# jneem/nnnoiseless

Hardware: NVIDIA H100
Metric: 48kHz mono frames/sec (480-sample) (higher is better)
Workload: dtype f32

## Files before the change

### nnnoiseless_b200/build.py

```python
import os
import subprocess
import sys

HERE = os.path.dirname(os.path.abspath(__file__))
CSRC = os.path.join(HERE, "csrc")
VARIANT = os.environ.get("NNB_VARIANT", "")
OBJ = os.path.join(HERE, "_obj" + ("_" + VARIANT if VARIANT else ""))
LIBDIR = os.path.join(HERE, "lib")
LIB = os.path.join(LIBDIR, "libnnnoiseless_b200%s.so" % ("_" + VARIANT if VARIANT else ""))
VARIANT_FLAGS = {"": [], "prof": ["-DPITCH_PROFILE", "-DRNN_TC_PROFILE"]}[VARIANT]
WEIGHTS = os.path.join(HERE, "data", "weights.rnn")
BINDIR = os.path.join(HERE, "bin")
CLI = os.path.join(BINDIR, "nnnoiseless-b200")
CLI_SRC = os.path.join(HERE, "..", "cli", "nnnoiseless_cli.cpp")
NVCC = os.environ.get("NVCC", "/usr/local/cuda/bin/nvcc")

ARCH = ["-gencode", "arch=compute_90a,code=sm_90a"]
COMMON = ["-O3", "-std=c++17", "-lineinfo", "-Xcompiler", "-fPIC", "-Xptxas", "-v"]

UNITS = [
    ("exact.cu", ["-fmad=false"]),
    ("pitch.cu", ["-fmad=false"]),
    ("train.cu", ["-fmad=false"]),
    ("spectral.cu", []),
    ("spectral_warp.cu", []),
    ("rnn.cu", ["-DRNN_RT=256", "-DRNN_UNROLL=8"]),
    ("rnn_mma.cu", []),
    ("rnn_tc.cu", []),
    ("frontend.cu", []),
    ("host.cu", []),
]
HEADERS = ["common.cuh", "fft480.cuh", "model.hpp", "audio_io.hpp", os.path.join("..", "..", "include", "rnnoise.h")]


def _newer(target, deps):
    if not os.path.exists(target):
        return True
    t = os.path.getmtime(target)
    return any(os.path.getmtime(d) > t for d in deps)


def build(force=False, verbose=False):
    os.makedirs(OBJ, exist_ok=True)
    os.makedirs(LIBDIR, exist_ok=True)
    hdrs = [os.path.join(CSRC, h) for h in HEADERS] + [os.path.abspath(__file__)]
    objs = []
    logs = []
    for src, extra in UNITS:
        s = os.path.join(CSRC, src)
        o = os.path.join(OBJ, src + ".o")
        objs.append(o)
        if force or _newer(o, [s] + hdrs):
            cmd = [NVCC] + ARCH + COMMON + extra + VARIANT_FLAGS + os.environ.get("NNB_EXTRA_NVCC", "").split() + ["-c", s, "-o", o]
            r = subprocess.run(cmd, capture_output=True, text=True)
            logs.append(r.stderr)
            if r.returncode != 0:
                sys.stderr.write(r.stdout + r.stderr)
                raise RuntimeError("nvcc failed on " + src)
            if verbose:
                sys.stderr.write(r.stderr)
    s = os.path.join(CSRC, "model.cpp")
    o = os.path.join(OBJ, "model.cpp.o")
    objs.append(o)
    if force or _newer(o, [s, WEIGHTS] + hdrs):
        cmd = ["g++", "-O2", "-std=c++17", "-fPIC", '-DNNB_WEIGHTS_PATH="%s"' % WEIGHTS, "-c", s, "-o", o]
        subprocess.run(cmd, check=True)
    s = os.path.join(CSRC, "audio_io.cpp")
    o = os.path.join(OBJ, "audio_io.cpp.o")
    objs.append(o)
    if force or _newer(o, [s] + hdrs):
        subprocess.run(["g++", "-O2", "-std=c++17", "-fPIC", "-Wall", "-c", s, "-o", o], check=True)
    if force or _newer(LIB, objs):
        cmd = [NVCC] + ARCH + ["-shared", "-o", LIB] + objs
        subprocess.run(cmd, check=True)
    os.makedirs(BINDIR, exist_ok=True)
    if not VARIANT and (force or _newer(CLI, [CLI_SRC, LIB] + hdrs)):
        cmd = ["g++", "-O2", "-std=c++17", "-Wall", CLI_SRC, "-o", CLI, "-L" + LIBDIR, "-lnnnoiseless_b200",
               "-Wl,-rpath,$ORIGIN/../lib"]
        subprocess.run(cmd, check=True)
    with open(os.path.join(OBJ, "ptxas.log"), "a") as f:
        f.write("".join(logs))
    return LIB


if __name__ == "__main__":
    print(build(force="--force" in sys.argv, verbose=True))
```

### nnnoiseless_b200/csrc/common.cuh

```cuda
#pragma once
#include <cuda_runtime.h>
#include <stdint.h>

namespace nnb {

constexpr int FRAME_SIZE = 480;
constexpr int WINDOW_SIZE = 960;
constexpr int FREQ_SIZE = 481;
constexpr int PITCH_MIN_PERIOD = 60;
constexpr int PITCH_MAX_PERIOD = 768;
constexpr int PITCH_FRAME_SIZE = 960;
constexpr int PITCH_BUF_SIZE = PITCH_MAX_PERIOD + PITCH_FRAME_SIZE;
constexpr int NB_BANDS = 22;
constexpr int CEPS_MEM = 8;
constexpr int NB_DELTA_CEPS = 6;
constexpr int NB_FEATURES = 42;
constexpr int MAX_NEURONS = 128;
constexpr int NB_BINS_BANDED = 400;
constexpr int BT_LANES = 96;

constexpr int HIST_SLOTS = 8;
constexpr int HIST_CAP = HIST_SLOTS * FRAME_SIZE;
constexpr int PIPE_DEPTH = 4;

__host__ __device__ inline int hist_base(int slot) { return (slot * FRAME_SIZE + (HIST_CAP - (PITCH_BUF_SIZE - FRAME_SIZE))) % HIST_CAP; }

struct DeviceTables {
    float window[WINDOW_SIZE];
    float dct[NB_BANDS * NB_BANDS];
    float wnorm;
    float tansig[201 + 3];
    float2 tw480[480];
    float2 tw960[FREQ_SIZE + 3];
    float band_frac[NB_BINS_BANDED];
    int32_t band_of[NB_BINS_BANDED];
    int32_t band_start[NB_BANDS];
    int16_t bt_bin[800];
    float bt_w[800];
    int16_t bt_lane_start[BT_LANES + 1];
    int16_t bt_band_lane[NB_BANDS + 1];
    int16_t bt_lane_band[BT_LANES];
    float2 twl[15][32];
    int16_t bp_seg[32];
    int16_t bp_b0[32];
    int16_t bp_n[32];
    int16_t bp_rot[32];
    int16_t bp_off[32];
    float bp_inv[32];
};
constexpr int BP_MAXBINS = 22;

struct DeviceLayer {
    int ni, nn, np, act;
    const float* w;
    const float* wh;
    const float* bias;
};

struct DeviceModel {
    DeviceLayer input_dense, vad_gru, noise_gru, denoise_gru, denoise_output, vad_output;
    int state_size;
};

constexpr int MMA_MAX_CHUNKS = 28;
struct MmaPhase {
    int nchunks;
    int ntiles;
    const uint2* wfrag;
    const float* bias;
    short col[MMA_MAX_CHUNKS];
};
struct DeviceModelMma {
    MmaPhase dense, vad_zr, vad_h, vad_out, noise_zr, noise_h, den_zr, den_h, out;
    int nd, nv, nn, ndn;
    int act_dense, act_vad, act_noise, act_den, act_out, act_vadout;
    int c_feat, c_dense, c_vad, c_noise, c_den, c_rh;
    int kp;
    int hs;
    int state_size;
};

struct BatchBuffers {
    int n_streams;
    float* hist;
    float* hp_mem;
    float* synth_mem;
    float* ceps_mem;
    int32_t* ceps_id;
    int32_t* last_period;
    float* last_gain;
    float* gru_state;
    float* lastg;
    float2* X;
    float2* P;
    float* ex;
    float* ep;
    float* exp;
    float* features;
    int32_t* silence;
    int32_t* pitch;
    float* gains;
    float* vad;
    unsigned long long* pitch_stats;
};

constexpr int TRAIN_ROW = NB_FEATURES + 2 * NB_BANDS + 1;
struct TrainLaneParams {
    float signal_gain, noise_gain;
    float sig_a[2], sig_b[2], noise_a[2], noise_b[2];
    int32_t band_lp;
};
struct TrainBuffers {
    int n_lanes;
    TrainLaneParams* params;
    float* resp_mem;
    int32_t* vad_count;
    float* vad;
    int32_t* cutoff;
};

struct DeviceGuard {
    int prev = -1, want = -1;
    cudaError_t err = cudaSuccess;
    explicit DeviceGuard(int dev) : want(dev) {
        err = cudaGetDevice(&prev);
        if (err == cudaSuccess && prev != dev) err = cudaSetDevice(dev);
    }
    ~DeviceGuard() {
        if (prev >= 0 && prev != want) cudaSetDevice(prev);
    }
    DeviceGuard(const DeviceGuard&) = delete;
    DeviceGuard& operator=(const DeviceGuard&) = delete;
};

cudaError_t launch_hp_filter(const BatchBuffers& b, const void* in, bool pcm16, long stream_stride, long sample_stride, int slot,
                             cudaStream_t st);
cudaError_t launch_pitch(const BatchBuffers& b, int slot, int force_exact, cudaStream_t st);
cudaError_t launch_analysis(const BatchBuffers& b, const DeviceTables* tab, int slot, cudaStream_t st);
cudaError_t launch_synthesis(const BatchBuffers& b, const DeviceTables* tab, void* out, bool pcm16, long stream_stride, long sample_stride,
                             float* vad_out, cudaStream_t st);
cudaError_t launch_analysis_warp(const BatchBuffers& b, const DeviceTables* tab, int slot, cudaStream_t st);
cudaError_t launch_synthesis_warp(const BatchBuffers& b, const DeviceTables* tab, void* out, bool pcm16, long stream_stride,
                                  long sample_stride, float* vad_out, cudaStream_t st);
cudaError_t launch_rnn(const BatchBuffers& b, const DeviceModel& m, const DeviceTables* tab, cudaStream_t st);
cudaError_t launch_rnn_mma(const BatchBuffers& b, const DeviceModelMma& m, const DeviceTables* tab, cudaStream_t st);

constexpr int TC_PHASES = 9;
enum { PH_DENSE = 0, PH_VAD_ZR, PH_VAD_H, PH_VAD_OUT, PH_NOISE_ZR, PH_NOISE_H, PH_DEN_ZR, PH_DEN_H, PH_OUT };
struct TcPhase {
    int n;
    int nk;
    uint32_t w_off;
    uint32_t b_off;
    short chunk[16];
};
constexpr int TC_MAX_SLABS = 64;
struct TcSlab {
    uint32_t off, bytes;
    short phase, kc0, kc1;
};
struct DeviceModelTc {
    TcPhase ph[TC_PHASES];
    int nd, nv, nn, ndn;
    int p_d, p_v, p_n, p_dn;
    int o_dense, o_vad, o_noise, o_den, o_rh;
    int act_dense, act_vad, act_noise, act_den, act_out, act_vadout;
    int state_size;
    const unsigned char* blob;
    uint32_t blob_bytes, table_off;
    int n_slabs;
    short slab0[TC_PHASES + 1];
    TcSlab slab[TC_MAX_SLABS];
};

struct UploadedTc {
    DeviceModelTc dm{};
    unsigned char* d_blob = nullptr;
    size_t smem_bytes = 0;
    bool ok = false;
};

struct HostModel;
int upload_model_tc(const HostModel& hm, UploadedTc* u, cudaStream_t st);
cudaError_t launch_rnn_tc(const BatchBuffers& b, const UploadedTc& u, cudaStream_t st);

cudaError_t launch_train_front(const BatchBuffers& b, const TrainBuffers& tb, int set, const float* signal, const float* noise,
                               long stream_stride, int slot, cudaStream_t st);
cudaError_t launch_train_rows(const BatchBuffers& b, const TrainBuffers& tb, int set, float* rows, long lane_stride, cudaStream_t st);

}
```

### nnnoiseless_b200/csrc/host.cu

```cuda
#include <atomic>
#include <cmath>
#include <cstdio>
#include <cstdlib>
#include <cstring>
#include <mutex>
#include <new>
#include <string>
#include <algorithm>
#include <utility>
#include <vector>

#include <cuda_fp16.h>

#include "../../include/rnnoise.h"
#include "common.cuh"
#include "model.hpp"

using namespace nnb;

struct RNNModel {
    HostModel m;
};

namespace {

thread_local std::string g_err;
std::atomic<unsigned long long> g_launches{0};

int fail(const std::string& what, cudaError_t e = cudaSuccess) {
    g_err = what;
    if (e != cudaSuccess) {
        g_err += ": ";
        g_err += cudaGetErrorString(e);
    }
    return -1;
}

}

namespace nnb {
int set_error(const std::string& what) { return fail(what); }
void count_launches(int n) { g_launches.fetch_add((unsigned long long)n, std::memory_order_relaxed); }
}

namespace {

#define ON_DEVICE(dev)                                                   \
    DeviceGuard guard__(dev);                                            \
    if (guard__.err != cudaSuccess) return fail("cudaSetDevice", guard__.err)

#define CK(call)                                         \
    do {                                                 \
        cudaError_t e__ = (call);                        \
        if (e__ != cudaSuccess) return fail(#call, e__); \
    } while (0)

}
namespace nnb {
extern const float kTansigTable[201] = {
    0.000000f, 0.039979f, 0.079830f, 0.119427f, 0.158649f, 0.197375f, 0.235496f, 0.272905f, 0.309507f, 0.345214f, 0.379949f,
    0.413644f, 0.446244f, 0.477700f, 0.507977f, 0.537050f, 0.564900f, 0.591519f, 0.616909f, 0.641077f, 0.664037f, 0.685809f,
    0.706419f, 0.725897f, 0.744277f, 0.761594f, 0.777888f, 0.793199f, 0.807569f, 0.821040f, 0.833655f, 0.845456f, 0.856485f,
    0.866784f, 0.876393f, 0.885352f, 0.893698f, 0.901468f, 0.908698f, 0.915420f, 0.921669f, 0.927473f, 0.932862f, 0.937863f,
    0.942503f, 0.946806f, 0.950795f, 0.954492f, 0.957917f, 0.961090f, 0.964028f, 0.966747f, 0.969265f, 0.971594f, 0.973749f,
    0.975743f, 0.977587f, 0.979293f, 0.980869f, 0.982327f, 0.983675f, 0.984921f, 0.986072f, 0.987136f, 0.988119f, 0.989027f,
    0.989867f, 0.990642f, 0.991359f, 0.992020f, 0.992631f, 0.993196f, 0.993718f, 0.994199f, 0.994644f, 0.995055f, 0.995434f,
    0.995784f, 0.996108f, 0.996407f, 0.996682f, 0.996937f, 0.997172f, 0.997389f, 0.997590f, 0.997775f, 0.997946f, 0.998104f,
    0.998249f, 0.998384f, 0.998508f, 0.998623f, 0.998728f, 0.998826f, 0.998916f, 0.999000f, 0.999076f, 0.999147f, 0.999213f,
    0.999273f, 0.999329f, 0.999381f, 0.999428f, 0.999472f, 0.999513f, 0.999550f, 0.999585f, 0.999617f, 0.999646f, 0.999673f,
    0.999699f, 0.999722f, 0.999743f, 0.999763f, 0.999781f, 0.999798f, 0.999813f, 0.999828f, 0.999841f, 0.999853f, 0.999865f,
    0.999875f, 0.999885f, 0.999893f, 0.999902f, 0.999909f, 0.999916f, 0.999923f, 0.999929f, 0.999934f, 0.999939f, 0.999944f,
    0.999948f, 0.999952f, 0.999956f, 0.999959f, 0.999962f, 0.999965f, 0.999968f, 0.999970f, 0.999973f, 0.999975f, 0.999977f,
    0.999978f, 0.999980f, 0.999982f, 0.999983f, 0.999984f, 0.999986f, 0.999987f, 0.999988f, 0.999989f, 0.999990f, 0.999990f,
    0.999991f, 0.999992f, 0.999992f, 0.999993f, 0.999994f, 0.999994f, 0.999994f, 0.999995f, 0.999995f, 0.999996f, 0.999996f,
    0.999996f, 0.999997f, 0.999997f, 0.999997f, 0.999997f, 0.999997f, 0.999998f, 0.999998f, 0.999998f, 0.999998f, 0.999998f,
    0.999998f, 0.999999f, 0.999999f, 0.999999f, 0.999999f, 0.999999f, 0.999999f, 0.999999f, 0.999999f, 0.999999f, 0.999999f,
    0.999999f, 0.999999f, 0.999999f, 1.000000f, 1.000000f, 1.000000f, 1.000000f, 1.000000f, 1.000000f, 1.000000f, 1.000000f,
    1.000000f, 1.000000f, 1.000000f,
};
}
namespace {
const int kEband5ms[NB_BANDS] = {0, 1, 2, 3, 4, 5, 6, 7, 8, 10, 12, 14, 16, 20, 24, 28, 34, 40, 48, 60, 78, 100};

void build_tables(DeviceTables* t) {
    std::memset(t, 0, sizeof(*t));
    const double pi = 3.14159265358979323846264338327950288;
    for (int i = 0; i < FRAME_SIZE; i++) {
        double s = std::sin(0.5 * pi * ((double)i + 0.5) / (double)FRAME_SIZE);
        float w = (float)std::sin(0.5 * pi * s * s);
        t->window[i] = w;
        t->window[WINDOW_SIZE - i - 1] = w;
    }
    volatile float acc = 0.0f;
    for (int i = 0; i < WINDOW_SIZE; i++) acc = acc + t->window[i] * t->window[i];
    t->wnorm = 1.0f / acc;
    for (int i = 0; i < NB_BANDS; i++)
        for (int j = 0; j < NB_BANDS; j++) {
            float v = (float)std::cos(((double)i + 0.5) * (double)j * pi / (double)NB_BANDS);
            if (j == 0) v *= std::sqrt(0.5f);
            t->dct[i * NB_BANDS + j] = v;
        }
    for (int i = 0; i < 201; i++) t->tansig[i] = kTansigTable[i];
    for (int k = 0; k < 480; k++)
        t->tw480[k] = make_float2((float)std::cos(-2.0 * pi * (double)k / 480.0), (float)std::sin(-2.0 * pi * (double)k / 480.0));
    for (int k = 0; k <= 480; k++)
        t->tw960[k] = make_float2((float)std::cos(-2.0 * pi * (double)k / 960.0), (float)std::sin(-2.0 * pi * (double)k / 960.0));
    for (int i = 0; i < NB_BANDS; i++) t->band_start[i] = kEband5ms[i] << 2;
    for (int i = 0; i < NB_BANDS - 1; i++) {
        int band_size = (kEband5ms[i + 1] - kEband5ms[i]) << 2;
        for (int j = 0; j < band_size; j++) {
            int idx = (kEband5ms[i] << 2) + j;
            t->band_frac[idx] = (float)j / (float)band_size;
            t->band_of[idx] = i;
        }
    }
    int nterm = 0, lane = 0;
    for (int b = 0; b < NB_BANDS; b++) {
        const int first = nterm;
        if (b > 0)
            for (int i = t->band_start[b - 1]; i < t->band_start[b]; i++) {
                t->bt_bin[nterm] = (int16_t)i;
                t->bt_w[nterm++] = t->band_frac[i];
            }
        if (b < NB_BANDS - 1)
            for (int i = t->band_start[b]; i < t->band_start[b + 1]; i++) {
                t->bt_bin[nterm] = (int16_t)i;
                t->bt_w[nterm++] = 1.0f - t->band_frac[i];
            }
        const int n = nterm - first, lanes = (n + 8) / 9;
        t->bt_band_lane[b] = (int16_t)lane;
        for (int l = 0; l < lanes; l++) {
            t->bt_lane_band[lane] = (int16_t)b;
            t->bt_lane_start[lane++] = (int16_t)(first + (int)((long)n * l / lanes));
        }
    }
    for (int k1 = 0; k1 < 15; k1++)
        for (int b = 0; b < 32; b++) {
            const double ang = -2.0 * pi * (double)(b * k1) / 480.0;
            t->twl[k1][b] = make_float2((float)std::cos(ang), (float)std::sin(ang));
        }
    {
        int l = 0;
        for (int sgi = 0; sgi < NB_BANDS - 1; sgi++) {
            const int first = t->band_start[sgi], size = t->band_start[sgi + 1] - first;
            const int nl = size <= 16 ? 1 : (size <= 32 ? 2 : (size <= 48 ? 3 : 4));
            for (int q = 0; q < nl; q++) {
                const int lo = first + (int)((long)size * q / nl), hi = first + (int)((long)size * (q + 1) / nl);
                if (l >= 32 || hi - lo > BP_MAXBINS) {
                    fprintf(stderr, "nnnoiseless_b200: band partition broken\n");
                    abort();
                }
                static const int kRot[32] = {2, 1, 0, 0, 3, 0, 1, 0, 6, 5, 4, 0, 1, 6, 3, 0, 9, 2, 0, 12, 2, 1, 15, 3, 15, 3, 2, 2, 21, 19, 12, 4};
                t->bp_seg[l] = (int16_t)sgi;
                t->bp_b0[l] = (int16_t)lo;
                t->bp_n[l] = (int16_t)(hi - lo);
                t->bp_rot[l] = (int16_t)(kRot[l] % (hi - lo));
                t->bp_off[l] = (int16_t)(lo - first);
                t->bp_inv[l] = 1.0f / (float)size;
                l++;
            }
        }
        if (l != 32) {
            fprintf(stderr, "nnnoiseless_b200: band partition uses %d lanes\n", l);
            abort();
        }
    }
    t->bt_band_lane[NB_BANDS] = (int16_t)lane;
    t->bt_lane_start[lane] = (int16_t)nterm;
    if (lane != BT_LANES || nterm != 800) {
        fprintf(stderr, "nnnoiseless_b200: band table construction broken (%d lanes, %d terms)\n", lane, nterm);
        abort();
    }
}

struct UploadedModel {
    DeviceModel dm{};
    float* d_blob = nullptr;
};

inline int pad4(int n) { return (n + 3) & ~3; }
size_t dense_floats(const HostDense& l) { return (size_t)l.ni * pad4(l.nn) + pad4(l.nn); }
size_t gru_floats(const HostGru& l) { return (size_t)(l.ni + l.nn) * 3 * pad4(l.nn) + 3 * pad4(l.nn); }

void fill_dense(const HostModel& m, const HostDense& l, std::vector<float>& blob, size_t* off, DeviceLayer* out, float* dbase) {
    const int8_t* w = m.bytes.data() + l.w_off;
    const int8_t* b = m.bytes.data() + l.b_off;
    const int np = pad4(l.nn);
    out->ni = l.ni;
    out->nn = l.nn;
    out->np = np;
    out->act = l.act;
    out->w = dbase + *off;
    for (int j = 0; j < l.ni; j++)
        for (int o = 0; o < np; o++) blob[(*off)++] = o < l.nn ? (float)w[(size_t)j * l.nn + o] : 0.0f;
    out->wh = nullptr;
    out->bias = dbase + *off;
    for (int o = 0; o < np; o++) blob[(*off)++] = o < l.nn ? (float)b[o] : 0.0f;
}

void fill_gru(const HostModel& m, const HostGru& l, std::vector<float>& blob, size_t* off, DeviceLayer* out, float* dbase) {
    const int8_t* w = m.bytes.data() + l.w_off;
    const int8_t* r = m.bytes.data() + l.r_off;
    const int8_t* b = m.bytes.data() + l.b_off;
    const int ni = l.ni, nn = l.nn, st = 3 * nn, np = pad4(nn);
    out->ni = ni;
    out->nn = nn;
    out->np = np;
    out->act = l.act;
    auto put_rows = [&](const int8_t* src, int rows, int gate0, int ngates) {
        for (int j = 0; j < rows; j++)
            for (int g = 0; g < ngates; g++)
                for (int o = 0; o < np; o++) blob[(*off)++] = o < nn ? (float)src[(size_t)j * st + (gate0 + g) * nn + o] : 0.0f;
    };
    out->w = dbase + *off;
    put_rows(w, ni, 0, 2);
    put_rows(r, nn, 0, 2);
    out->wh = dbase + *off;
    put_rows(w, ni, 2, 1);
    put_rows(r, nn, 2, 1);
    out->bias = dbase + *off;
    for (int g = 0; g < 3; g++)
        for (int o = 0; o < np; o++) blob[(*off)++] = o < nn ? (float)b[g * nn + o] : 0.0f;
}

int upload_model(const HostModel& m, UploadedModel* um, cudaStream_t st) {
    size_t total = dense_floats(m.input_dense) + gru_floats(m.vad_gru) + gru_floats(m.noise_gru) + gru_floats(m.denoise_gru) +
                   dense_floats(m.denoise_output) + dense_floats(m.vad_output);
    std::vector<float> blob(total);
    CK(cudaMalloc(&um->d_blob, total * sizeof(float)));
    size_t off = 0;
    fill_dense(m, m.input_dense, blob, &off, &um->dm.input_dense, um->d_blob);
    fill_gru(m, m.vad_gru, blob, &off, &um->dm.vad_gru, um->d_blob);
    fill_gru(m, m.noise_gru, blob, &off, &um->dm.noise_gru, um->d_blob);
    fill_gru(m, m.denoise_gru, blob, &off, &um->dm.denoise_gru, um->d_blob);
    fill_dense(m, m.denoise_output, blob, &off, &um->dm.denoise_output, um->d_blob);
    fill_dense(m, m.vad_output, blob, &off, &um->dm.vad_output, um->d_blob);
    um->dm.state_size = m.vad_gru.nn + m.noise_gru.nn + m.denoise_gru.nn;
    CK(cudaMemcpyAsync(um->d_blob, blob.data(), total * sizeof(float), cudaMemcpyHostToDevice, st));
    CK(cudaStreamSynchronize(st));
    return 0;
}

struct UploadedMma {
    DeviceModelMma dm{};
    unsigned char* d_blob = nullptr;
};

struct Seg {
    int acol, len, recurrent, src_off;
};

inline int pad16(int n) { return (n + 15) & ~15; }
inline uint32_t pack_h2(int a, int b) {
    return (uint32_t)__half_as_ushort(__float2half((float)a)) | ((uint32_t)__half_as_ushort(__float2half((float)b)) << 16);
}

struct PhaseBuilder {
    std::vector<unsigned char> blob;
    std::vector<std::pair<MmaPhase*, std::pair<size_t, size_t>>> fixups;

    template <typename WF, typename BF>
    void add(MmaPhase* ph, const std::vector<Seg>& segs, int nout, int ngates, WF weight, BF bias) {
        const int ot = (nout + 7) / 8;
        ph->ntiles = ngates * ot;
        ph->nchunks = 0;
        std::vector<std::pair<int, int>> chunks;
        for (size_t si = 0; si < segs.size(); si++)
            for (int c = 0; c < pad16(segs[si].len); c += 16) {
                if (ph->nchunks >= MMA_MAX_CHUNKS) abort();
                ph->col[ph->nchunks++] = (short)(segs[si].acol + c);
                chunks.push_back({(int)si, c});
            }
        while (blob.size() % 16) blob.push_back(0);
        const size_t woff = blob.size();
        blob.resize(woff + (size_t)ph->nchunks * ph->ntiles * 32 * sizeof(uint2));
        uint2* wf = reinterpret_cast<uint2*>(blob.data() + woff);
        for (int kc = 0; kc < ph->nchunks; kc++) {
            const Seg& sg = segs[chunks[kc].first];
            const int r0 = chunks[kc].second;
            for (int nt = 0; nt < ph->ntiles; nt++) {
                const int gate = nt / ot, o0 = (nt % ot) * 8;
                for (int lane = 0; lane < 32; lane++) {
                    const int g = lane >> 2, t = lane & 3, n = o0 + g;
                    auto w = [&](int kr) -> int {
                        const int i = r0 + kr;
                        if (i >= sg.len || n >= nout) return 0;
                        return weight(sg, i, gate, n);
                    };
                    wf[((size_t)kc * ph->ntiles + nt) * 32 + lane] =
                        make_uint2(pack_h2(w(2 * t), w(2 * t + 1)), pack_h2(w(2 * t + 8), w(2 * t + 9)));
                }
            }
        }
        const size_t boff = blob.size();
        blob.resize(boff + (size_t)ph->ntiles * 8 * sizeof(float));
        float* bf = reinterpret_cast<float*>(blob.data() + boff);
        for (int nt = 0; nt < ph->ntiles; nt++)
            for (int j = 0; j < 8; j++) {
                const int gate = nt / ot, o = (nt % ot) * 8 + j;
                bf[nt * 8 + j] = o < nout ? (float)bias(gate, o) : 0.0f;
            }
        fixups.push_back({ph, {woff, boff}});
    }
};

int upload_model_mma(const HostModel& m, UploadedMma* um, cudaStream_t st) {
    DeviceModelMma& d = um->dm;
    const int nd = m.input_dense.nn, nv = m.vad_gru.nn, nn = m.noise_gru.nn, ndn = m.denoise_gru.nn;
    d.nd = nd; d.nv = nv; d.nn = nn; d.ndn = ndn;
    d.act_dense = m.input_dense.act; d.act_vad = m.vad_gru.act; d.act_noise = m.noise_gru.act; d.act_den = m.denoise_gru.act;
    d.act_out = m.denoise_output.act; d.act_vadout = m.vad_output.act;
    d.c_feat = 0;
    d.c_dense = pad16(NB_FEATURES);
    d.c_vad = d.c_dense + pad16(nd);
    d.c_noise = d.c_vad + pad16(nv);
    d.c_den = d.c_noise + pad16(nn);
    d.c_rh = d.c_den + pad16(ndn);
    int cols = d.c_rh + pad16(std::max(nv, std::max(nn, ndn)));
    int kp = cols;
    while ((kp / 2) % 8 != 4) kp += 2;
    d.kp = kp;
    int hs = ((nv + 7) & ~7) + ((nn + 7) & ~7) + ((ndn + 7) & ~7);
    while (hs % 32 != 8) hs++;
    d.hs = hs;
    d.state_size = nv + nn + ndn;

    const int8_t* B = m.bytes.data();
    PhaseBuilder pb;
    auto dense_w = [&](const HostDense& L) {
        return [&, B](const Seg& sg, int i, int, int n) -> int { return B[L.w_off + (size_t)(sg.src_off + i) * L.nn + n]; };
    };
    auto dense_b = [&](const HostDense& L) { return [&, B](int, int o) -> int { return B[L.b_off + o]; }; };
    auto gru_w = [&](const HostGru& L, int gate0) {
        return [&, B, gate0](const Seg& sg, int i, int gate, int n) -> int {
            const size_t st3 = (size_t)3 * L.nn;
            const size_t base = sg.recurrent ? L.r_off : L.w_off;
            return B[base + (size_t)(sg.src_off + i) * st3 + (size_t)(gate0 + gate) * L.nn + n];
        };
    };
    auto gru_b = [&](const HostGru& L, int gate0) { return [&, B, gate0](int gate, int o) -> int { return B[L.b_off + (size_t)(gate0 + gate) * L.nn + o]; }; };

    pb.add(&d.dense, {{d.c_feat, NB_FEATURES, 0, 0}}, nd, 1, dense_w(m.input_dense), dense_b(m.input_dense));
    pb.add(&d.vad_zr, {{d.c_dense, nd, 0, 0}, {d.c_vad, nv, 1, 0}}, nv, 2, gru_w(m.vad_gru, 0), gru_b(m.vad_gru, 0));
    pb.add(&d.vad_h, {{d.c_dense, nd, 0, 0}, {d.c_rh, nv, 1, 0}}, nv, 1, gru_w(m.vad_gru, 2), gru_b(m.vad_gru, 2));
    pb.add(&d.vad_out, {{d.c_vad, nv, 0, 0}}, 1, 1, dense_w(m.vad_output), dense_b(m.vad_output));
    pb.add(&d.noise_zr, {{d.c_dense, nd, 0, 0}, {d.c_vad, nv, 0, nd}, {d.c_feat, NB_FEATURES, 0, nd + nv}, {d.c_noise, nn, 1, 0}}, nn, 2,
           gru_w(m.noise_gru, 0), gru_b(m.noise_gru, 0));
    pb.add(&d.noise_h, {{d.c_dense, nd, 0, 0}, {d.c_vad, nv, 0, nd}, {d.c_feat, NB_FEATURES, 0, nd + nv}, {d.c_rh, nn, 1, 0}}, nn, 1,
           gru_w(m.noise_gru, 2), gru_b(m.noise_gru, 2));
    pb.add(&d.den_zr, {{d.c_vad, nv, 0, 0}, {d.c_noise, nn, 0, nv}, {d.c_feat, NB_FEATURES, 0, nv + nn}, {d.c_den, ndn, 1, 0}}, ndn, 2,
           gru_w(m.denoise_gru, 0), gru_b(m.denoise_gru, 0));
    pb.add(&d.den_h, {{d.c_vad, nv, 0, 0}, {d.c_noise, nn, 0, nv}, {d.c_feat, NB_FEATURES, 0, nv + nn}, {d.c_rh, ndn, 1, 0}}, ndn, 1,
           gru_w(m.denoise_gru, 2), gru_b(m.denoise_gru, 2));
    pb.add(&d.out, {{d.c_den, ndn, 0, 0}}, NB_BANDS, 1, dense_w(m.denoise_output), dense_b(m.denoise_output));

    CK(cudaMalloc(&um->d_blob, pb.blob.size()));
    for (auto& f : pb.fixups) {
        f.first->wfrag = reinterpret_cast<const uint2*>(um->d_blob + f.second.first);
        f.first->bias = reinterpret_cast<const float*>(um->d_blob + f.second.second);
    }
    CK(cudaMemcpyAsync(um->d_blob, pb.blob.data(), pb.blob.size(), cudaMemcpyHostToDevice, st));
    CK(cudaStreamSynchronize(st));
    return 0;
}

}

constexpr int kNumKernels = 5;
const char* const kKernelNames[kNumKernels] = {"hp_filter", "pitch", "analysis", "rnn", "synthesis"};
constexpr int kEvRing = 16;

struct RNNoiseBatch {
    int device = 0;
    int n_streams = 0;
    cudaStream_t st[kNumKernels] = {nullptr, nullptr, nullptr, nullptr, nullptr};
    cudaStream_t c_in = nullptr, c_out = nullptr;
    cudaEvent_t ev[kNumKernels][kEvRing];
    cudaEvent_t ev_in[kEvRing], ev_call = nullptr;
    bool events_ok = false;
    BatchBuffers buf{};
    std::vector<void*> allocs;
    DeviceTables* d_tab = nullptr;
    UploadedModel um;
    UploadedMma umm;
    UploadedTc utc;
    bool rnn_mma = false;
    bool rnn_fp32 = false;
    bool spectral_v1 = false;
    bool serial = false;
    int pitch_exact = 0;
    unsigned long long frame = 0;
    char* stage_in = nullptr;
    char* stage_out = nullptr;
    float* stage_vad = nullptr;
    size_t stage_bytes = 0;
    cudaEvent_t ev_out[8];
    int slot_ev[8];
};
constexpr int kStageSlots = 8;

namespace {

template <typename T>
int dalloc(RNNoiseBatch* b, T** p, size_t count) {
    void* q = nullptr;
    CK(cudaMalloc(&q, count * sizeof(T)));
    b->allocs.push_back(q);
    *p = reinterpret_cast<T*>(q);
    return 0;
}

BatchBuffers view(const RNNoiseBatch* b, unsigned long long f) {
    BatchBuffers v = b->buf;
    const size_t k = (size_t)(f % PIPE_DEPTH), B = (size_t)b->n_streams;
    v.X += k * B * FREQ_SIZE;
    v.P += k * B * NB_BINS_BANDED;
    v.ex += k * B * NB_BANDS;
    v.ep += k * B * NB_BANDS;
    v.exp += k * B * NB_BANDS;
    v.features += k * B * NB_FEATURES;
    v.silence += k * B;
    v.pitch += k * B;
    v.gains += k * B * NB_BANDS;
    v.vad += k * B;
    return v;
}

int sync_all(RNNoiseBatch* b) {
    for (int i = 0; i < kNumKernels; i++) CK(cudaStreamSynchronize(b->st[i]));
    CK(cudaStreamSynchronize(b->c_in));
    CK(cudaStreamSynchronize(b->c_out));
    return 0;
}

int zero_state(RNNoiseBatch* b) {
    const size_t B = (size_t)b->n_streams, D = PIPE_DEPTH;
    BatchBuffers& u = b->buf;
    const int SS = b->um.dm.state_size;
    if (sync_all(b)) return -1;
    cudaStream_t s = b->st[0];
    CK(cudaMemsetAsync(u.hist, 0, B * HIST_CAP * sizeof(float), s));
    CK(cudaMemsetAsync(u.hp_mem, 0, B * 2 * sizeof(float), s));
    CK(cudaMemsetAsync(u.synth_mem, 0, B * FRAME_SIZE * sizeof(float), s));
    CK(cudaMemsetAsync(u.ceps_mem, 0, B * CEPS_MEM * NB_BANDS * sizeof(float), s));
    CK(cudaMemsetAsync(u.ceps_id, 0, B * sizeof(int32_t), s));
    CK(cudaMemsetAsync(u.last_period, 0, B * sizeof(int32_t), s));
    CK(cudaMemsetAsync(u.last_gain, 0, B * sizeof(float), s));
    CK(cudaMemsetAsync(u.gru_state, 0, B * SS * sizeof(float), s));
    CK(cudaMemsetAsync(u.lastg, 0, B * NB_BANDS * sizeof(float), s));
    CK(cudaMemsetAsync(u.gains, 0, D * B * NB_BANDS * sizeof(float), s));
    CK(cudaMemsetAsync(u.vad, 0, D * B * sizeof(float), s));
    CK(cudaMemsetAsync(u.silence, 0, D * B * sizeof(int32_t), s));
    CK(cudaMemsetAsync(u.pitch, 0, D * B * sizeof(int32_t), s));
    CK(cudaMemsetAsync(u.features, 0, D * B * NB_FEATURES * sizeof(float), s));
    b->frame = 0;
    CK(cudaStreamSynchronize(s));
    return 0;
}

int batch_init(RNNoiseBatch* b, const HostModel& hm, int n_streams, int device) {
    int ndev = 0;
    cudaError_t e = cudaGetDeviceCount(&ndev);
    if (e != cudaSuccess || ndev == 0) return fail("no CUDA device available (this library has no CPU fallback)", e);
    if (device < 0) CK(cudaGetDevice(&device));
    if (device >= ndev) return fail("device index out of range");
    if (n_streams <= 0) return fail("n_streams must be positive");
    CK(cudaSetDevice(device));
    b->device = device;
    b->n_streams = n_streams;
    for (int i = 0; i < kNumKernels; i++) CK(cudaStreamCreateWithFlags(&b->st[i], cudaStreamNonBlocking));
    CK(cudaStreamCreateWithFlags(&b->c_in, cudaStreamNonBlocking));
    CK(cudaStreamCreateWithFlags(&b->c_out, cudaStreamNonBlocking));
    for (int i = 0; i < kNumKernels; i++)
        for (int k = 0; k < kEvRing; k++) CK(cudaEventCreateWithFlags(&b->ev[i][k], cudaEventDisableTiming));
    for (int k = 0; k < kEvRing; k++) CK(cudaEventCreateWithFlags(&b->ev_in[k], cudaEventDisableTiming));
    CK(cudaEventCreateWithFlags(&b->ev_call, cudaEventDisableTiming));
    for (int k = 0; k < kStageSlots; k++) CK(cudaEventCreateWithFlags(&b->ev_out[k], cudaEventDisableTiming));
    b->events_ok = true;
    const size_t B = (size_t)n_streams, D = PIPE_DEPTH;
    BatchBuffers& u = b->buf;
    u.n_streams = n_streams;
    if (upload_model(hm, &b->um, b->st[0])) return -1;
    b->allocs.push_back(b->um.d_blob);
    if (upload_model_mma(hm, &b->umm, b->st[0])) return -1;
    b->allocs.push_back(b->umm.d_blob);
    if (upload_model_tc(hm, &b->utc, b->st[0])) return fail("tensor-core model upload");
    if (b->utc.d_blob) b->allocs.push_back(b->utc.d_blob);
    {
        const char* e1 = getenv("NNB_RNN_FP32");
        b->rnn_fp32 = e1 && e1[0] == '1';
        const char* e2 = getenv("NNB_SERIAL");
        b->serial = e2 && e2[0] == '1';
        const char* e5 = getenv("NNB_RNN_MMA");
        b->rnn_mma = e5 && e5[0] == '1';
        const char* e4 = getenv("NNB_SPECTRAL_V1");
        b->spectral_v1 = e4 && e4[0] == '1';
        const char* e3 = getenv("NNB_PITCH_EXACT");
        b->pitch_exact = !e3 ? 0 : (e3[0] == '1' ? 3 : (e3[0] == '2' ? 1 : (e3[0] == '3' ? 2 : 0)));
    }
    const int SS = b->um.dm.state_size;
    if (dalloc(b, &u.hist, B * HIST_CAP) || dalloc(b, &u.hp_mem, B * 2) || dalloc(b, &u.synth_mem, B * FRAME_SIZE) ||
        dalloc(b, &u.ceps_mem, B * CEPS_MEM * NB_BANDS) || dalloc(b, &u.ceps_id, B) || dalloc(b, &u.last_period, B) ||
        dalloc(b, &u.last_gain, B) || dalloc(b, &u.gru_state, B * SS) || dalloc(b, &u.lastg, B * NB_BANDS) ||
        dalloc(b, &u.X, D * B * FREQ_SIZE) || dalloc(b, &u.P, D * B * NB_BINS_BANDED) || dalloc(b, &u.ex, D * B * NB_BANDS) ||
        dalloc(b, &u.ep, D * B * NB_BANDS) || dalloc(b, &u.exp, D * B * NB_BANDS) || dalloc(b, &u.features, D * B * NB_FEATURES) ||
        dalloc(b, &u.silence, D * B) || dalloc(b, &u.pitch, D * B) || dalloc(b, &u.gains, D * B * NB_BANDS) ||
        dalloc(b, &u.vad, D * B) || dalloc(b, &b->d_tab, 1) || dalloc(b, &u.pitch_stats, 3))
        return -1;
    CK(cudaMemsetAsync(u.pitch_stats, 0, 3 * sizeof(unsigned long long), b->st[0]));
    DeviceTables* ht = new DeviceTables();
    build_tables(ht);
    cudaError_t ce = cudaMemcpyAsync(b->d_tab, ht, sizeof(DeviceTables), cudaMemcpyHostToDevice, b->st[0]);
    if (ce == cudaSuccess) ce = cudaStreamSynchronize(b->st[0]);
    delete ht;
    if (ce != cudaSuccess) return fail("table upload", ce);
    return zero_state(b);
}

void free_stage(RNNoiseBatch* b) {
    if (b->stage_in) cudaFree(b->stage_in);
    if (b->stage_out) cudaFree(b->stage_out);
    if (b->stage_vad) cudaFree(b->stage_vad);
    b->stage_in = b->stage_out = nullptr;
    b->stage_vad = nullptr;
    b->stage_bytes = 0;
}

void batch_release(RNNoiseBatch* b) {
    if (!b) return;
    DeviceGuard guard(b->device);
    for (int i = 0; i < kNumKernels; i++)
        if (b->st[i]) cudaStreamSynchronize(b->st[i]);
    if (b->c_in) cudaStreamSynchronize(b->c_in);
    if (b->c_out) cudaStreamSynchronize(b->c_out);
    for (void* p : b->allocs) cudaFree(p);
    b->allocs.clear();
    free_stage(b);
    if (b->events_ok) {
        for (int i = 0; i < kNumKernels; i++)
            for (int k = 0; k < kEvRing; k++) cudaEventDestroy(b->ev[i][k]);
        for (int k = 0; k < kEvRing; k++) cudaEventDestroy(b->ev_in[k]);
        for (int k = 0; k < kStageSlots; k++) cudaEventDestroy(b->ev_out[k]);
        cudaEventDestroy(b->ev_call);
        b->events_ok = false;
    }
    for (int i = 0; i < kNumKernels; i++)
        if (b->st[i]) {
            cudaStreamDestroy(b->st[i]);
            b->st[i] = nullptr;
        }
    if (b->c_in) cudaStreamDestroy(b->c_in);
    if (b->c_out) cudaStreamDestroy(b->c_out);
    b->c_in = b->c_out = nullptr;
}

int ensure_stage(RNNoiseBatch* b, bool pcm) {
    const size_t need = (size_t)kStageSlots * b->n_streams * FRAME_SIZE * (pcm ? sizeof(short) : sizeof(float));
    if (need > b->stage_bytes) {
        if (sync_all(b)) return -1;
        free_stage(b);
        CK(cudaMalloc(&b->stage_in, need));
        CK(cudaMalloc(&b->stage_out, need));
        CK(cudaMalloc(&b->stage_vad, (size_t)kStageSlots * b->n_streams * sizeof(float)));
        b->stage_bytes = need;
    }
    return 0;
}

constexpr int kFmtF32 = 0, kFmtPcmIn = 1, kFmtPcmOut = 2, kFmtPcm = 3;
int launch_stage(RNNoiseBatch* b, int i, const BatchBuffers& v, void* out, const void* in, int fmt, float* vad, long stream_stride,
                 long sample_stride, int slot, cudaStream_t s) {
    switch (i) {
        case 0: CK(launch_hp_filter(v, in, (fmt & kFmtPcmIn) != 0, stream_stride, sample_stride, slot, s)); break;
        case 1: CK(launch_pitch(v, slot, b->pitch_exact, s)); break;
        case 2:
            if (b->spectral_v1) CK(launch_analysis(v, b->d_tab, slot, s));
            else CK(launch_analysis_warp(v, b->d_tab, slot, s));
            break;
        case 3:
            if (b->rnn_fp32) CK(launch_rnn(v, b->um.dm, b->d_tab, s));
            else if (b->utc.ok && !b->rnn_mma) CK(launch_rnn_tc(v, b->utc, s));
            else CK(launch_rnn_mma(v, b->umm.dm, b->d_tab, s));
            break;
        default:
            if (b->spectral_v1) CK(launch_synthesis(v, b->d_tab, out, (fmt & kFmtPcmOut) != 0, stream_stride, sample_stride, vad, s));
            else CK(launch_synthesis_warp(v, b->d_tab, out, (fmt & kFmtPcmOut) != 0, stream_stride, sample_stride, vad, s));
            break;
    }
    return 0;
}

int step_serial(RNNoiseBatch* b, void* out, const void* in, int fmt, float* vad, long stream_stride, long sample_stride, cudaStream_t s,
                cudaEvent_t* tev = nullptr) {
    const int slot = (int)(b->frame % HIST_SLOTS);
    const BatchBuffers v = view(b, b->frame);
    for (int i = 0; i < kNumKernels; i++) {
        if (tev) CK(cudaEventRecord(tev[i], s));
        if (launch_stage(b, i, v, out, in, fmt, vad, stream_stride, sample_stride, slot, s)) return -1;
    }
    if (tev) CK(cudaEventRecord(tev[kNumKernels], s));
    g_launches.fetch_add(kNumKernels, std::memory_order_relaxed);
    b->frame++;
    return 0;
}

int step_pipelined(RNNoiseBatch* b, void* out, const void* in, int fmt, float* vad, long stream_stride, long sample_stride,
                   cudaEvent_t in_ready) {
    const unsigned long long f = b->frame;
    const int slot = (int)(f % HIST_SLOTS), e = (int)(f % kEvRing);
    const BatchBuffers v = view(b, f);
    if (in_ready) CK(cudaStreamWaitEvent(b->st[0], in_ready, 0));
    if (f >= (unsigned long long)PIPE_DEPTH) CK(cudaStreamWaitEvent(b->st[0], b->ev[kNumKernels - 1][(int)((f - PIPE_DEPTH) % kEvRing)], 0));
    for (int i = 0; i < kNumKernels; i++) {
        if (i > 0) CK(cudaStreamWaitEvent(b->st[i], b->ev[i - 1][e], 0));
        if (launch_stage(b, i, v, out, in, fmt, vad, stream_stride, sample_stride, slot, b->st[i])) return -1;
        CK(cudaEventRecord(b->ev[i][e], b->st[i]));
    }
    g_launches.fetch_add(kNumKernels, std::memory_order_relaxed);
    b->frame++;
    return 0;
}

int join_into(RNNoiseBatch* b, cudaStream_t s) {
    if (b->frame == 0) return 0;
    CK(cudaStreamWaitEvent(s, b->ev[kNumKernels - 1][(int)((b->frame - 1) % kEvRing)], 0));
    return 0;
}

}

extern "C" {

const char* rnnoise_last_error(void) { return g_err.c_str(); }
unsigned long long rnnoise_kernel_launches(void) { return g_launches.load(); }

RNNModel* rnnoise_model_from_bytes(const unsigned char* bytes, size_t len) {
    RNNModel* m = new (std::nothrow) RNNModel();
    if (!m) return nullptr;
    if (!bytes || !HostModel::parse(bytes, len, &m->m)) {
        delete m;
        fail("model bytes rejected (src/rnn.rs:116-232 validation)");
        return nullptr;
    }
    return m;
}

RNNModel* rnnoise_model_from_text(const char* text, size_t len) {
    RNNModel* m = new (std::nothrow) RNNModel();
    if (!m) return nullptr;
    if (!text || !HostModel::parse_text(text, len, &m->m)) {
        delete m;
        fail("text model rejected");
        return nullptr;
    }
    return m;
}

RNNModel* rnnoise_model_from_file(FILE* file) {
    if (!file) return nullptr;
    std::vector<unsigned char> data;
    unsigned char chunk[65536];
    size_t n;
    bool err = false;
    while ((n = fread(chunk, 1, sizeof chunk, file)) > 0) data.insert(data.end(), chunk, chunk + n);
    if (ferror(file)) err = true;
    fclose(file);
    if (err) return nullptr;
    return rnnoise_model_from_bytes(data.data(), data.size());
}

void rnnoise_model_free(RNNModel* model) { delete model; }

size_t rnnoise_model_bytes(const RNNModel* model, unsigned char* buf, size_t cap) {
    const HostModel& m = model ? model->m : HostModel::builtin();
    if (buf && cap >= m.bytes.size()) std::memcpy(buf, m.bytes.data(), m.bytes.size());
    return m.bytes.size();
}

RNNoiseBatch* rnnoise_batch_create(const RNNModel* model, int n_streams, int device) {
    RNNoiseBatch* b = new (std::nothrow) RNNoiseBatch();
    if (!b) return nullptr;
    const HostModel& hm = model ? model->m : HostModel::builtin();
    int prev_dev = -1;
    cudaGetDevice(&prev_dev);
    const int rc = batch_init(b, hm, n_streams, device);
    if (prev_dev >= 0) cudaSetDevice(prev_dev);
    if (rc != 0) {
        std::string keep = g_err;
        batch_release(b);
        delete b;
        g_err = keep;
        return nullptr;
    }
    return b;
}

void rnnoise_batch_destroy(RNNoiseBatch* b) {
    if (!b) return;
    batch_release(b);
    delete b;
}

int rnnoise_batch_streams(const RNNoiseBatch* b) { return b ? b->n_streams : 0; }

int rnnoise_batch_reset(RNNoiseBatch* b) {
    if (!b) return fail("null batch");
    ON_DEVICE(b->device);
    return zero_state(b);
}

static int process_device_impl(RNNoiseBatch* b, void* out, const void* in, int fmt, float* vad, int n_frames, long stream_stride,
                               long sample_stride, long frame_stride, void* cuda_stream) {
    if (!b || !out || !in) return fail("null argument");
    if (sample_stride < 1) return fail("sample_stride must be >= 1");
    if (n_frames < 0) return fail("negative n_frames");
    if (n_frames == 0) return 0;
    ON_DEVICE(b->device);
    if (fmt < 0 || fmt > 3) return fail("pcm16 must be 0..3");
    const size_t esz_in = (fmt & kFmtPcmIn) ? sizeof(short) : sizeof(float), esz_out = (fmt & kFmtPcmOut) ? sizeof(short) : sizeof(float);
    auto at_in = [&](const void* p, int t) { return (const void*)((const char*)p + (size_t)t * frame_stride * esz_in); };
    auto at_out = [&](void* p, int t) { return (void*)((char*)p + (size_t)t * frame_stride * esz_out); };
    cudaStream_t us = (cudaStream_t)cuda_stream;
    if (b->serial) {
        cudaStream_t s = us ? us : b->st[0];
        for (int t = 0; t < n_frames; t++)
            if (step_serial(b, at_out(out, t), at_in(in, t), fmt, vad ? vad + (size_t)t * b->n_streams : nullptr, stream_stride, sample_stride, s))
                return -1;
        if (!us) CK(cudaStreamSynchronize(s));
        return 0;
    }
    cudaEvent_t ready = nullptr;
    if (us) {
        CK(cudaEventRecord(b->ev_call, us));
        ready = b->ev_call;
    }
    for (int t = 0; t < n_frames; t++) {
        if (step_pipelined(b, at_out(out, t), at_in(in, t), fmt, vad ? vad + (size_t)t * b->n_streams : nullptr, stream_stride, sample_stride,
                           t == 0 ? ready : nullptr))
            return -1;
    }
    if (us) {
        if (join_into(b, us)) return -1;
    } else {
        CK(cudaStreamSynchronize(b->st[kNumKernels - 1]));
    }
    return 0;
}

int rnnoise_batch_process_device(RNNoiseBatch* b, float* out, const float* in, float* vad, int n_frames, long stream_stride,
                                 long frame_stride, void* cuda_stream) {
    return process_device_impl(b, out, in, kFmtF32, vad, n_frames, stream_stride, 1, frame_stride, cuda_stream);
}

int rnnoise_batch_process_device_pcm16(RNNoiseBatch* b, short* out, const short* in, float* vad, int n_frames, long stream_stride,
                                       long frame_stride, void* cuda_stream) {
    return process_device_impl(b, out, in, kFmtPcm, vad, n_frames, stream_stride, 1, frame_stride, cuda_stream);
}

int rnnoise_batch_process_device_strided(RNNoiseBatch* b, void* out, const void* in, int pcm16, float* vad, int n_frames, long stream_stride,
                                         long sample_stride, long frame_stride, void* cuda_stream) {
    if (pcm16 < 0 || pcm16 > 3) return fail("pcm16 must be 0..3");
    static const int to_fmt[4] = {kFmtF32, kFmtPcm, kFmtPcmOut, kFmtPcmIn};
    return process_device_impl(b, out, in, to_fmt[pcm16], vad, n_frames, stream_stride, sample_stride, frame_stride, cuda_stream);
}

const char* rnnoise_kernel_name(int i) { return (i >= 0 && i < kNumKernels) ? kKernelNames[i] : nullptr; }

int rnnoise_batch_profile_step(RNNoiseBatch* b, float* out, const float* in, float* vad, long stream_stride, void* cuda_stream,
                               float* ms, int cap) {
    if (!b || !out || !in || !ms) return fail("null argument");
    if (cap < kNumKernels) return fail("ms[] too small");
    ON_DEVICE(b->device);
    if (sync_all(b)) return -1;
    cudaStream_t st = cuda_stream ? (cudaStream_t)cuda_stream : b->st[0];
    cudaEvent_t ev[kNumKernels + 1];
    for (int i = 0; i <= kNumKernels; i++) CK(cudaEventCreate(&ev[i]));
    int rc = step_serial(b, out, in, kFmtF32, vad, stream_stride, 1, st, ev);
    if (rc == 0) {
        cudaError_t e = cudaStreamSynchronize(st);
        if (e != cudaSuccess) rc = fail("profile_step sync", e);
    }
    if (rc == 0)
        for (int i = 0; i < kNumKernels; i++) cudaEventElapsedTime(&ms[i], ev[i], ev[i + 1]);
    for (int i = 0; i <= kNumKernels; i++) cudaEventDestroy(ev[i]);
    if (rc == 0) {
        const int e = (int)((b->frame - 1) % kEvRing);
        for (int i = 0; i < kNumKernels; i++) cudaEventRecord(b->ev[i][e], st);
        cudaStreamSynchronize(st);
    }
    return rc == 0 ? kNumKernels : rc;
}

static int process_host_impl(RNNoiseBatch* b, void* out, const void* in, bool pcm, float* vad, int n_frames) {
    if (ensure_stage(b, pcm)) return -1;
    const size_t B = (size_t)b->n_streams, fs = B * FRAME_SIZE;
    const size_t esz = pcm ? sizeof(short) : sizeof(float);
    char* din = b->stage_in;
    char* dout = b->stage_out;
    const int last = kNumKernels - 1;
    if (join_into(b, b->c_in)) return -1;
    for (int t = 0; t < n_frames; t++) {
        const int e = (int)(b->frame % kEvRing), k = t % kStageSlots;
        cudaStream_t first_st = b->st[0], last_st = b->serial ? b->st[0] : b->st[last];
        if (t >= kStageSlots) {
            CK(cudaStreamWaitEvent(b->c_in, b->serial ? b->ev[last][b->slot_ev[k]] : b->ev[0][b->slot_ev[k]], 0));
            CK(cudaStreamWaitEvent(last_st, b->ev_out[k], 0));
        }
        CK(cudaMemcpyAsync(din + k * fs * esz, (const char*)in + (size_t)t * fs * esz, fs * esz, cudaMemcpyHostToDevice, b->c_in));
        CK(cudaEventRecord(b->ev_in[e], b->c_in));
        if (b->serial) {
            CK(cudaStreamWaitEvent(first_st, b->ev_in[e], 0));
            if (step_serial(b, dout + k * fs * esz, din + k * fs * esz, pcm ? kFmtPcm : kFmtF32, b->stage_vad + (size_t)k * B, FRAME_SIZE, 1, first_st)) return -1;
            CK(cudaEventRecord(b->ev[last][e], first_st));
        } else {
            if (step_pipelined(b, dout + k * fs * esz, din + k * fs * esz, pcm ? kFmtPcm : kFmtF32, b->stage_vad + (size_t)k * B, FRAME_SIZE, 1, b->ev_in[e])) return -1;
        }
        CK(cudaStreamWaitEvent(b->c_out, b->ev[last][e], 0));
        CK(cudaMemcpyAsync((char*)out + (size_t)t * fs * esz, dout + k * fs * esz, fs * esz, cudaMemcpyDeviceToHost, b->c_out));
        if (vad) CK(cudaMemcpyAsync(vad + (size_t)t * B, b->stage_vad + (size_t)k * B, B * sizeof(float), cudaMemcpyDeviceToHost, b->c_out));
        CK(cudaEventRecord(b->ev_out[k], b->c_out));
        b->slot_ev[k] = e;
    }
    CK(cudaStreamSynchronize(b->c_out));
    CK(cudaStreamSynchronize(b->c_in));
    return 0;
}

int rnnoise_batch_process_host(RNNoiseBatch* b, float* out, const float* in, float* vad, int n_frames) {
    if (!b || !out || !in) return fail("null argument");
    if (n_frames <= 0) return n_frames == 0 ? 0 : fail("negative n_frames");
    ON_DEVICE(b->device);
    return process_host_impl(b, out, in, false, vad, n_frames);
}

int rnnoise_batch_process_pcm16_host(RNNoiseBatch* b, short* out, const short* in, float* vad, int n_frames) {
    if (!b || !out || !in) return fail("null argument");
    if (n_frames <= 0) return n_frames == 0 ? 0 : fail("negative n_frames");
    ON_DEVICE(b->device);
    return process_host_impl(b, out, in, true, vad, n_frames);
}

int rnnoise_batch_pitch_stats(RNNoiseBatch* b, unsigned long long out[3]) {
    if (!b || !out) return fail("null argument");
    ON_DEVICE(b->device);
    if (sync_all(b)) return -1;
    CK(cudaMemcpy(out, b->buf.pitch_stats, 3 * sizeof(unsigned long long), cudaMemcpyDeviceToHost));
    return 0;
}

int rnnoise_batch_get_taps(RNNoiseBatch* b, int* pitch, int* silence, float* features, float* gains) {
    if (!b) return fail("null batch");
    ON_DEVICE(b->device);
    const size_t B = (size_t)b->n_streams;
    if (sync_all(b)) return -1;
    const BatchBuffers v = view(b, b->frame ? b->frame - 1 : 0);
    if (pitch) CK(cudaMemcpy(pitch, v.pitch, B * sizeof(int), cudaMemcpyDeviceToHost));
    if (silence) CK(cudaMemcpy(silence, v.silence, B * sizeof(int), cudaMemcpyDeviceToHost));
    if (features) CK(cudaMemcpy(features, v.features, B * NB_FEATURES * sizeof(float), cudaMemcpyDeviceToHost));
    if (gains) CK(cudaMemcpy(gains, v.lastg, B * NB_BANDS * sizeof(float), cudaMemcpyDeviceToHost));
    return 0;
}

int rnnoise_batch_get_rnn_taps(RNNoiseBatch* b, float* gains, float* vad, float* gru_state) {
    if (!b) return fail("null batch");
    ON_DEVICE(b->device);
    const size_t B = (size_t)b->n_streams;
    if (sync_all(b)) return -1;
    const BatchBuffers v = view(b, b->frame ? b->frame - 1 : 0);
    if (gains) CK(cudaMemcpy(gains, v.gains, B * NB_BANDS * sizeof(float), cudaMemcpyDeviceToHost));
    if (vad) CK(cudaMemcpy(vad, v.vad, B * sizeof(float), cudaMemcpyDeviceToHost));
    if (gru_state) CK(cudaMemcpy(gru_state, v.gru_state, B * b->um.dm.state_size * sizeof(float), cudaMemcpyDeviceToHost));
    return 0;
}

}

static_assert(sizeof(RNNoiseSimParams) == sizeof(TrainLaneParams), "C ABI struct and device struct must match");
constexpr int kTrainStages = 4;

struct RNNoiseTrainer {
    RNNoiseBatch* batch = nullptr;
    TrainBuffers tb{};
    float* stage_sig = nullptr;
    float* stage_noise = nullptr;
    float* stage_rows = nullptr;
    int stage_frames = 0;
};

namespace {

void trainer_release(RNNoiseTrainer* t) {
    if (!t) return;
    DeviceGuard guard(t->batch ? t->batch->device : 0);
    if (t->batch) sync_all(t->batch);
    cudaFree(t->tb.params);
    cudaFree(t->tb.resp_mem);
    cudaFree(t->tb.vad_count);
    cudaFree(t->tb.vad);
    cudaFree(t->tb.cutoff);
    cudaFree(t->stage_sig);
    cudaFree(t->stage_noise);
    cudaFree(t->stage_rows);
    if (t->batch) rnnoise_batch_destroy(t->batch);
    delete t;
}

int trainer_init(RNNoiseTrainer* t, int n_lanes) {
    const size_t L = (size_t)n_lanes;
    TrainBuffers& tb = t->tb;
    tb.n_lanes = n_lanes;
    CK(cudaMalloc(&tb.params, L * sizeof(TrainLaneParams)));
    CK(cudaMalloc(&tb.resp_mem, L * 4 * sizeof(float)));
    CK(cudaMalloc(&tb.vad_count, L * sizeof(int32_t)));
    CK(cudaMalloc(&tb.vad, PIPE_DEPTH * L * sizeof(float)));
    CK(cudaMalloc(&tb.cutoff, PIPE_DEPTH * L * sizeof(int32_t)));
    CK(cudaMemset(tb.resp_mem, 0, L * 4 * sizeof(float)));
    CK(cudaMemset(tb.vad_count, 0, L * sizeof(int32_t)));
    TrainLaneParams d{};
    d.signal_gain = 1.0f;
    d.noise_gain = 1.0f;
    d.band_lp = NB_BANDS - 1;
    std::vector<TrainLaneParams> init(L, d);
    CK(cudaMemcpy(tb.params, init.data(), L * sizeof(TrainLaneParams), cudaMemcpyHostToDevice));
    return 0;
}

int train_step(RNNoiseTrainer* t, float* rows, long row_lane_stride, const float* sig, const float* noise, long stream_stride,
               cudaEvent_t in_ready) {
    RNNoiseBatch* b = t->batch;
    const unsigned long long f = b->frame;
    const int slot = (int)(f % HIST_SLOTS), e = (int)(f % kEvRing), set = (int)(f % PIPE_DEPTH);
    const BatchBuffers v = view(b, f);
    cudaStream_t s0 = b->serial ? b->st[0] : nullptr;
    auto S = [&](int i) { return s0 ? s0 : b->st[i]; };
    if (in_ready) CK(cudaStreamWaitEvent(S(0), in_ready, 0));
    if (!s0 && f >= (unsigned long long)PIPE_DEPTH) CK(cudaStreamWaitEvent(S(0), b->ev[kTrainStages - 1][(int)((f - PIPE_DEPTH) % kEvRing)], 0));
    for (int i = 0; i < kTrainStages; i++) {
        if (!s0 && i > 0) CK(cudaStreamWaitEvent(S(i), b->ev[i - 1][e], 0));
        switch (i) {
            case 0: CK(launch_train_front(v, t->tb, set, sig, noise, stream_stride, slot, S(i))); break;
            case 1: CK(launch_pitch(v, slot, b->pitch_exact, S(i))); break;
            case 2:
                if (b->spectral_v1) CK(launch_analysis(v, b->d_tab, slot, S(i)));
                else CK(launch_analysis_warp(v, b->d_tab, slot, S(i)));
                break;
            default: CK(launch_train_rows(v, t->tb, set, rows, row_lane_stride, S(i))); break;
        }
        CK(cudaEventRecord(b->ev[i][e], S(i)));
    }
    g_launches.fetch_add(kTrainStages, std::memory_order_relaxed);
    b->frame++;
    return 0;
}

int train_join(RNNoiseTrainer* t, cudaStream_t s) {
    RNNoiseBatch* b = t->batch;
    if (b->frame == 0) return 0;
    CK(cudaStreamWaitEvent(s, b->ev[kTrainStages - 1][(int)((b->frame - 1) % kEvRing)], 0));
    return 0;
}

}

extern "C" {

RNNoiseTrainer* rnnoise_train_create(int n_lanes, int device) {
    if (n_lanes <= 0 || n_lanes > (1 << 29) / 3) {
        fail("n_lanes out of range");
        return nullptr;
    }
    RNNoiseTrainer* t = new (std::nothrow) RNNoiseTrainer();
    if (!t) return nullptr;
    t->batch = rnnoise_batch_create(nullptr, 3 * n_lanes, device);
    int trc = -1;
    if (t->batch) {
        DeviceGuard guard(t->batch->device);
        trc = guard.err == cudaSuccess ? trainer_init(t, n_lanes) : fail("cudaSetDevice", guard.err);
    }
    if (!t->batch || trc != 0) {
        std::string keep = g_err;
        trainer_release(t);
        g_err = keep;
        return nullptr;
    }
    return t;
}

void rnnoise_train_destroy(RNNoiseTrainer* t) { trainer_release(t); }
int rnnoise_train_lanes(const RNNoiseTrainer* t) { return t ? t->tb.n_lanes : 0; }

int rnnoise_train_band_lp(int lowpass) {
    static const int eband[NB_BANDS] = {0, 1, 2, 3, 4, 5, 6, 7, 8, 10, 12, 14, 16, 20, 24, 28, 34, 40, 48, 60, 78, 100};
    for (int i = 0; i < NB_BANDS; i++)
        if ((eband[i] << 2) > lowpass) return i;
    return NB_BANDS - 1;
}

int rnnoise_train_set_params(RNNoiseTrainer* t, int first_lane, int n, const RNNoiseSimParams* params) {
    if (!t || !params) return fail("null argument");
    if (first_lane < 0 || n < 0 || first_lane + n > t->tb.n_lanes) return fail("lane range out of bounds");
    for (int i = 0; i < n; i++)
        if (params[i].band_lp < 0 || params[i].band_lp >= NB_BANDS) return fail("band_lp must be in [0, 21]");
    ON_DEVICE(t->batch->device);
    if (sync_all(t->batch)) return -1;
    CK(cudaMemcpy(t->tb.params + first_lane, params, (size_t)n * sizeof(TrainLaneParams), cudaMemcpyHostToDevice));
    return 0;
}

int rnnoise_train_process_device(RNNoiseTrainer* t, float* rows, const float* signal, const float* noise, int n_frames, long stream_stride,
                                 long frame_stride, long row_lane_stride, long row_frame_stride, void* cuda_stream) {
    if (!t || !rows || !signal || !noise) return fail("null argument");
    if (n_frames < 0) return fail("negative n_frames");
    if (n_frames == 0) return 0;
    RNNoiseBatch* b = t->batch;
    ON_DEVICE(b->device);
    cudaStream_t us = (cudaStream_t)cuda_stream;
    cudaEvent_t ready = nullptr;
    if (us) {
        CK(cudaEventRecord(b->ev_call, us));
        ready = b->ev_call;
    }
    for (int f = 0; f < n_frames; f++)
        if (train_step(t, rows + (size_t)f * row_frame_stride, row_lane_stride, signal + (size_t)f * frame_stride,
                       noise + (size_t)f * frame_stride, stream_stride, f == 0 ? ready : nullptr))
            return -1;
    cudaStream_t last = b->serial ? b->st[0] : b->st[kTrainStages - 1];
    if (us) {
        if (train_join(t, us)) return -1;
    } else {
        CK(cudaStreamSynchronize(last));
    }
    return 0;
}

int rnnoise_train_process_host(RNNoiseTrainer* t, float* rows, const float* signal, const float* noise, int n_frames) {
    if (!t || !rows || !signal || !noise) return fail("null argument");
    if (n_frames < 0) return fail("negative n_frames");
    if (n_frames == 0) return 0;
    RNNoiseBatch* b = t->batch;
    ON_DEVICE(b->device);
    const size_t L = (size_t)t->tb.n_lanes;
    const int chunk = (int)std::max<size_t>(1, std::min<size_t>((size_t)n_frames, (size_t(256) << 20) / (L * FRAME_SIZE * sizeof(float))));
    if (chunk > t->stage_frames) {
        if (sync_all(b)) return -1;
        cudaFree(t->stage_sig);
        cudaFree(t->stage_noise);
        cudaFree(t->stage_rows);
        t->stage_sig = t->stage_noise = t->stage_rows = nullptr;
        t->stage_frames = 0;
        CK(cudaMalloc(&t->stage_sig, (size_t)chunk * L * FRAME_SIZE * sizeof(float)));
        CK(cudaMalloc(&t->stage_noise, (size_t)chunk * L * FRAME_SIZE * sizeof(float)));
        CK(cudaMalloc(&t->stage_rows, (size_t)chunk * L * TRAIN_ROW * sizeof(float)));
        t->stage_frames = chunk;
    }
    for (int f0 = 0; f0 < n_frames; f0 += chunk) {
        const int nf = std::min(chunk, n_frames - f0);
        const size_t off = (size_t)f0 * L;
        CK(cudaMemcpyAsync(t->stage_sig, signal + off * FRAME_SIZE, (size_t)nf * L * FRAME_SIZE * sizeof(float), cudaMemcpyHostToDevice, b->c_in));
        CK(cudaMemcpyAsync(t->stage_noise, noise + off * FRAME_SIZE, (size_t)nf * L * FRAME_SIZE * sizeof(float), cudaMemcpyHostToDevice, b->c_in));
        if (rnnoise_train_process_device(t, t->stage_rows, t->stage_sig, t->stage_noise, nf, FRAME_SIZE, (long)(L * FRAME_SIZE), TRAIN_ROW,
                                         (long)(L * TRAIN_ROW), b->c_in))
            return -1;
        CK(cudaMemcpyAsync(rows + off * TRAIN_ROW, t->stage_rows, (size_t)nf * L * TRAIN_ROW * sizeof(float), cudaMemcpyDeviceToHost, b->c_in));
        CK(cudaStreamSynchronize(b->c_in));
    }
    return 0;
}

}

extern "C" {

struct DenoiseState {
    RNNoiseBatch* batch;
};

int rnnoise_get_frame_size(void) { return FRAME_SIZE; }
int rnnoise_get_size(void) { return (int)sizeof(DenoiseState); }

int rnnoise_init(DenoiseState* st, RNNModel* model) {
    if (!st) return fail("null state");
    st->batch = rnnoise_batch_create(model, 1, -1);
    return st->batch ? 0 : -1;
}

DenoiseState* rnnoise_create(RNNModel* model) {
    DenoiseState* st = new (std::nothrow) DenoiseState();
    if (!st) return nullptr;
    if (rnnoise_init(st, model) != 0) {
        delete st;
        return nullptr;
    }
    return st;
}

void rnnoise_destroy(DenoiseState* st) {
    if (!st) return;
    rnnoise_batch_destroy(st->batch);
    delete st;
}

float rnnoise_process_frame(DenoiseState* st, float* out, float* in) {
    if (!st || !st->batch) {
        fprintf(stderr, "rnnoise_process_frame: Invalid pointer\n");
        abort();
    }
    float vad = 0.0f;
    if (rnnoise_batch_process_host(st->batch, out, in, &vad, 1) != 0) {
        fprintf(stderr, "rnnoise_process_frame: %s\n", g_err.c_str());
        abort();
    }
    return vad;
}

}
```

### nnnoiseless_b200/csrc/spectral.cu

```cuda
#include "common.cuh"

namespace nnb {

constexpr int ST = 128;

__device__ __forceinline__ float2 cmul(float2 a, float2 b) { return make_float2(a.x * b.x - a.y * b.y, a.x * b.y + a.y * b.x); }
__device__ __forceinline__ float2 cadd(float2 a, float2 b) { return make_float2(a.x + b.x, a.y + b.y); }
__device__ __forceinline__ float2 csub(float2 a, float2 b) { return make_float2(a.x - b.x, a.y - b.y); }

template <int R>
__device__ __forceinline__ void butterfly(float2* a) {
    if (R == 2) {
        float2 t = a[0];
        a[0] = cadd(t, a[1]);
        a[1] = csub(t, a[1]);
    } else if (R == 4) {
        float2 t0 = cadd(a[0], a[2]), t1 = csub(a[0], a[2]);
        float2 t2 = cadd(a[1], a[3]), t3 = csub(a[1], a[3]);
        a[0] = cadd(t0, t2);
        a[1] = make_float2(t1.x + t3.y, t1.y - t3.x);
        a[2] = csub(t0, t2);
        a[3] = make_float2(t1.x - t3.y, t1.y + t3.x);
    } else if (R == 3) {
        const float s = 0.86602540378443864676f;
        float2 t1 = cadd(a[1], a[2]), d = csub(a[1], a[2]);
        float2 m1 = make_float2(a[0].x - 0.5f * t1.x, a[0].y - 0.5f * t1.y);
        a[0] = cadd(a[0], t1);
        a[1] = make_float2(m1.x + s * d.y, m1.y - s * d.x);
        a[2] = make_float2(m1.x - s * d.y, m1.y + s * d.x);
    } else if (R == 6) {
        const float h = 0.5f, s = 0.86602540378443864676f;
        float2 e[3] = {a[0], a[2], a[4]}, o[3] = {a[1], a[3], a[5]};
        butterfly<3>(e);
        butterfly<3>(o);
        const float2 t1 = make_float2(h * o[1].x + s * o[1].y, h * o[1].y - s * o[1].x);
        const float2 t2 = make_float2(s * o[2].y - h * o[2].x, -h * o[2].y - s * o[2].x);
        a[0] = cadd(e[0], o[0]);
        a[3] = csub(e[0], o[0]);
        a[1] = cadd(e[1], t1);
        a[4] = csub(e[1], t1);
        a[2] = cadd(e[2], t2);
        a[5] = csub(e[2], t2);
    } else if (R == 5) {
        const float c1 = 0.30901699437494742410f, c2 = -0.80901699437494742410f;
        const float s1 = 0.95105651629515357212f, s2 = 0.58778525229247312917f;
        float2 t1 = cadd(a[1], a[4]), t2 = cadd(a[2], a[3]);
        float2 d1 = csub(a[1], a[4]), d2 = csub(a[2], a[3]);
        float2 u1 = make_float2(a[0].x + c1 * t1.x + c2 * t2.x, a[0].y + c1 * t1.y + c2 * t2.y);
        float2 u2 = make_float2(a[0].x + c2 * t1.x + c1 * t2.x, a[0].y + c2 * t1.y + c1 * t2.y);
        float2 v1 = make_float2(s1 * d1.x + s2 * d2.x, s1 * d1.y + s2 * d2.y);
        float2 v2 = make_float2(s2 * d1.x - s1 * d2.x, s2 * d1.y - s1 * d2.y);
        a[0] = cadd(a[0], cadd(t1, t2));
        a[1] = make_float2(u1.x + v1.y, u1.y - v1.x);
        a[4] = make_float2(u1.x - v1.y, u1.y + v1.x);
        a[2] = make_float2(u2.x + v2.y, u2.y - v2.x);
        a[3] = make_float2(u2.x - v2.y, u2.y + v2.x);
    }
}

template <int R, int N, int S>
__device__ __forceinline__ void stockham_pass(const float2* __restrict__ x, float2* __restrict__ y,
                                              const float2* __restrict__ tw) {
    constexpr int M = N / R;
    for (int b = threadIdx.x; b < 480 / R; b += ST) {
        const int p = b / S, q = b - p * S;
        float2 a[R];
#pragma unroll
        for (int k = 0; k < R; k++) a[k] = x[q + S * (p + k * M)];
        butterfly<R>(a);
        y[q + S * (R * p)] = a[0];
#pragma unroll
        for (int j = 1; j < R; j++) {
            y[q + S * (R * p + j)] = (N == R) ? a[j] : cmul(a[j], __ldg(&tw[j * p * S]));
        }
    }
    __syncthreads();
}

__device__ void fft480(float2* a, float2* b, const float2* tw) {
    stockham_pass<4, 480, 1>(a, b, tw);
    stockham_pass<4, 120, 4>(b, a, tw);
    stockham_pass<5, 30, 16>(a, b, tw);
    stockham_pass<6, 6, 80>(b, a, tw);
}

template <int R, int N, int S>
__device__ __forceinline__ void stockham_pass2(const float2* __restrict__ x0, float2* __restrict__ y0, const float2* __restrict__ x1,
                                               float2* __restrict__ y1, const float2* __restrict__ tw) {
    constexpr int M = N / R;
    for (int b = threadIdx.x; b < 480 / R; b += ST) {
        const int p = b / S, q = b - p * S;
        float2 a[R], c[R];
#pragma unroll
        for (int k = 0; k < R; k++) {
            a[k] = x0[q + S * (p + k * M)];
            c[k] = x1[q + S * (p + k * M)];
        }
        butterfly<R>(a);
        butterfly<R>(c);
        y0[q + S * (R * p)] = a[0];
        y1[q + S * (R * p)] = c[0];
#pragma unroll
        for (int j = 1; j < R; j++) {
            if (N == R) {
                y0[q + S * (R * p + j)] = a[j];
                y1[q + S * (R * p + j)] = c[j];
            } else {
                const float2 w = __ldg(&tw[j * p * S]);
                y0[q + S * (R * p + j)] = cmul(a[j], w);
                y1[q + S * (R * p + j)] = cmul(c[j], w);
            }
        }
    }
    __syncthreads();
}
__device__ void fft480x2(float2* a0, float2* b0, float2* a1, float2* b1, const float2* tw) {
    stockham_pass2<4, 480, 1>(a0, b0, a1, b1, tw);
    stockham_pass2<4, 120, 4>(b0, a0, b1, a1, tw);
    stockham_pass2<5, 30, 16>(a0, b0, a1, b1, tw);
    stockham_pass2<6, 6, 80>(b0, a0, b1, a1, tw);
}

template <int NS>
__device__ __forceinline__ void band_sums(const float2* xs, const float2* ps, const DeviceTables* __restrict__ tab, float* part,
                                          float* o0, float* o1, float* o2) {
    const int tid = threadIdx.x, lane = tid & 31, warp = tid >> 5;
    static_assert(BT_LANES == 96, "three warps of band lanes");
    if (tid < BT_LANES) {
        const int t0 = tab->bt_lane_start[tid], n = tab->bt_lane_start[tid + 1] - t0;
        const int bin0 = tab->bt_bin[t0];
        const int band = tab->bt_lane_band[tid];
        float a0 = 0.0f, a1 = 0.0f, a2 = 0.0f;
#pragma unroll
        for (int i = 0; i < 9; i++) {
            if (i < n) {
                const float w = __ldg(&tab->bt_w[t0 + i]);
                const float2 x = xs[bin0 + i];
                a0 = fmaf(w, x.x * x.x + x.y * x.y, a0);
                if (NS == 3) {
                    const float2 p = ps[bin0 + i];
                    a1 = fmaf(w, p.x * p.x + p.y * p.y, a1);
                    a2 = fmaf(w, x.x * p.x + x.y * p.y, a2);
                }
            }
        }
#pragma unroll
        for (int off = 1; off < 32; off <<= 1) {
            const int ob = __shfl_down_sync(0xffffffffu, band, off);
            const float v0 = __shfl_down_sync(0xffffffffu, a0, off);
            const float v1 = NS == 3 ? __shfl_down_sync(0xffffffffu, a1, off) : 0.0f;
            const float v2 = NS == 3 ? __shfl_down_sync(0xffffffffu, a2, off) : 0.0f;
            if (lane + off < 32 && ob == band) {
                a0 += v0;
                if (NS == 3) {
                    a1 += v1;
                    a2 += v2;
                }
            }
        }
        const int prev = __shfl_up_sync(0xffffffffu, band, 1);
        if (lane == 0 || prev != band) {
            part[warp * NB_BANDS + band] = a0;
            if (NS == 3) {
                part[(3 + warp) * NB_BANDS + band] = a1;
                part[(6 + warp) * NB_BANDS + band] = a2;
            }
        }
    }
    __syncthreads();
    if (tid < NS * 32) {
        const int which = tid >> 5, b = tid & 31;
        if (b < NB_BANDS) {
            const int w0 = tab->bt_band_lane[b] >> 5, w1 = (tab->bt_band_lane[b + 1] - 1) >> 5;
            float acc = 0.0f;
            for (int w = w0; w <= w1; w++) acc += part[(which * 3 + w) * NB_BANDS + b];
            if (b == 0 || b == NB_BANDS - 1) acc *= 2.0f;
            float* o = which == 0 ? o0 : (which == 1 ? o1 : o2);
            o[b] = acc;
        }
    }
    __syncthreads();
}

__device__ __forceinline__ float interp_gain(const float* g, const DeviceTables* __restrict__ tab, int idx) {
    if (idx >= NB_BINS_BANDED) return 0.0f;
    int b = tab->band_of[idx];
    float f = tab->band_frac[idx];
    return (1.0f - f) * g[b] + f * g[b + 1];
}

struct WindowLoad {
    float4 hv[2], wv[2];
    float2 hs[4], ws[4];
    bool aligned;
    __device__ __forceinline__ void issue_loads(const float* __restrict__ h, int start, const DeviceTables* __restrict__ tab) {
        aligned = (start & 3) == 0;
        if (aligned) {
#pragma unroll
            for (int it = 0; it < 2; it++) {
                const int q = threadIdx.x + it * ST;
                hv[it] = make_float4(0.f, 0.f, 0.f, 0.f);
                wv[it] = hv[it];
                if (q < WINDOW_SIZE / 4) {
                    int pos = start + 4 * q;
                    if (pos >= HIST_CAP) pos -= HIST_CAP;
                    hv[it] = __ldg(reinterpret_cast<const float4*>(h + pos));
                    wv[it] = __ldg(reinterpret_cast<const float4*>(tab->window) + q);
                }
            }
        } else {
#pragma unroll
            for (int it = 0; it < 4; it++) {
                const int n = threadIdx.x + it * ST;
                hs[it] = make_float2(0.f, 0.f);
                ws[it] = hs[it];
                if (n < 480) {
                    int p0 = start + 2 * n;
                    if (p0 >= HIST_CAP) p0 -= HIST_CAP;
                    int p1 = p0 + 1;
                    if (p1 >= HIST_CAP) p1 -= HIST_CAP;
                    hs[it] = make_float2(__ldg(h + p0), __ldg(h + p1));
                    ws[it] = __ldg(reinterpret_cast<const float2*>(tab->window) + n);
                }
            }
        }
    }
    __device__ __forceinline__ void store(float2* a) const {
        if (aligned) {
#pragma unroll
            for (int it = 0; it < 2; it++) {
                const int q = threadIdx.x + it * ST;
                if (q < WINDOW_SIZE / 4)
                    reinterpret_cast<float4*>(a)[q] = make_float4(hv[it].x * wv[it].x, hv[it].y * wv[it].y, hv[it].z * wv[it].z, hv[it].w * wv[it].w);
            }
        } else {
#pragma unroll
            for (int it = 0; it < 4; it++) {
                const int n = threadIdx.x + it * ST;
                if (n < 480) a[n] = make_float2(hs[it].x * ws[it].x, hs[it].y * ws[it].y);
            }
        }
    }
};

__device__ __forceinline__ void rfft_post(const float2* b, float2* xs, const DeviceTables* __restrict__ tab) {
    const float wn = tab->wnorm;
#pragma unroll
    for (int it = 0; it < 2; it++) {
        const int k = threadIdx.x + it * ST;
        if (k <= 240) {
            const float2 zk = b[k], zc = b[k == 0 ? 0 : 480 - k];
            const float er = 0.5f * (zk.x + zc.x), ei = 0.5f * (zk.y - zc.y);
            const float dr = 0.5f * (zk.x - zc.x), di = 0.5f * (zk.y + zc.y);
            const float2 tw = __ldg(&tab->tw960[k]);
            const float tx = di * tw.x + dr * tw.y, ty = di * tw.y - dr * tw.x;
            float2 r0 = make_float2((er + tx) * wn, (ei + ty) * wn);
            float2 r1 = make_float2((er - tx) * wn, (ty - ei) * wn);
            if (k == 0) {
                r0.y = 0.0f;
                r1.y = 0.0f;
            }
            xs[k] = r0;
            if (k != 240) xs[480 - k] = r1;
        }
    }
}

__global__ void __launch_bounds__(ST, 10) analysis_kernel(BatchBuffers bb, const DeviceTables* __restrict__ tab, int hbase) {
    __shared__ __align__(16) float2 xa[FREQ_SIZE + 1];
    __shared__ __align__(16) float2 xb[480];
    __shared__ __align__(16) float2 pa[FREQ_SIZE + 1];
    __shared__ __align__(16) float2 pb[480];
    __shared__ float part[3 * BT_LANES];
    __shared__ float s_ex[NB_BANDS], s_ep[NB_BANDS], s_exp[NB_BANDS];
    __shared__ float s_feat[NB_FEATURES];
    __shared__ float s_ceps[CEPS_MEM][NB_BANDS];
    __shared__ float s_dist[CEPS_MEM][CEPS_MEM];

    const int s = blockIdx.x, tid = threadIdx.x;
    const float* h = bb.hist + (size_t)s * HIST_CAP;
    const int pitch = bb.pitch[s];

    int start = hbase + (PITCH_BUF_SIZE - WINDOW_SIZE);
    if (start >= HIST_CAP) start -= HIST_CAP;
    WindowLoad wx, wp;
    wx.issue_loads(h, start, tab);
    start = hbase + (PITCH_BUF_SIZE - WINDOW_SIZE) - pitch;
    if (start >= HIST_CAP) start -= HIST_CAP;
    wp.issue_loads(h, start, tab);
    wx.store(xa);
    wp.store(pa);
    __syncthreads();
    fft480x2(xa, xb, pa, pb, tab->tw480);
    float2* xs = xa;
    float2* ps = pa;
    rfft_post(xa, xs, tab);
    rfft_post(pa, ps, tab);
    __syncthreads();

    float2* Xg = bb.X + (size_t)s * FREQ_SIZE;
    float2* Pg = bb.P + (size_t)s * NB_BINS_BANDED;
    for (int k = tid; k <= 480; k += ST) Xg[k] = xs[k];
    for (int k = tid; k < NB_BINS_BANDED; k += ST) Pg[k] = ps[k];
    band_sums<3>(xs, ps, tab, part, s_ex, s_ep, s_exp);

    if (tid >= 32) return;
    const int lane = tid;
    const bool bl = lane < NB_BANDS;
    const float ex = bl ? s_ex[lane] : 0.0f, ep = bl ? s_ep[lane] : 0.0f;
    const float xpn = bl ? s_exp[lane] / sqrtf(0.001f + ex * ep) : 0.0f;
    if (bl) {
        bb.ex[(size_t)s * NB_BANDS + lane] = ex;
        bb.ep[(size_t)s * NB_BANDS + lane] = ep;
        bb.exp[(size_t)s * NB_BANDS + lane] = xpn;
    }
    float* cg = bb.ceps_mem + (size_t)s * CEPS_MEM * NB_BANDS;
    const int mem_id = bb.ceps_id[s];
    float cr[6];
#pragma unroll
    for (int k = 0; k < 6; k++) cr[k] = (lane + 32 * k < CEPS_MEM * NB_BANDS) ? cg[lane + 32 * k] : 0.0f;
    const float lg = bl ? log10f(1e-2f + ex) : 0.0f;
    float ly = 0.0f, log_max = -2.0f, follow = -2.0f, e = 0.0f;
#pragma unroll
    for (int k = 0; k < NB_BANDS; k++) {
        const float v = fmaxf(fmaxf(__shfl_sync(0xffffffffu, lg, k), log_max - 7.0f), follow - 1.5f);
        if (lane == k) ly = v;
        log_max = fmaxf(log_max, v);
        follow = fmaxf(follow - 1.5f, v);
        e += __shfl_sync(0xffffffffu, ex, k);
    }
    float* featg = bb.features + (size_t)s * NB_FEATURES;
    if (e < 0.04f) {
        featg[lane] = 0.0f;
        if (lane + 32 < NB_FEATURES) featg[lane + 32] = 0.0f;
        if (lane == 0) bb.silence[s] = 1;
        return;
    }
    const double dct_scale = 0.30151134457776362265;
    float sum_ly = 0.0f, sum_xp = 0.0f;
#pragma unroll
    for (int j = 0; j < NB_BANDS; j++) {
        const float d = bl ? __ldg(&tab->dct[j * NB_BANDS + lane]) : 0.0f;
        sum_ly += __shfl_sync(0xffffffffu, ly, j) * d;
        sum_xp += __shfl_sync(0xffffffffu, xpn, j) * d;
    }
    float ceps = (float)((double)sum_ly * dct_scale);
    float pcor = (float)((double)sum_xp * dct_scale);
    if (lane == 0) {
        ceps -= 12.0f;
        pcor -= 1.3f;
    }
    if (lane == 1) {
        ceps -= 4.0f;
        pcor -= 0.9f;
    }
#pragma unroll
    for (int k = 0; k < 6; k++)
        if (lane + 32 * k < CEPS_MEM * NB_BANDS) (&s_ceps[0][0])[lane + 32 * k] = cr[k];
    __syncwarp();
    if (bl) {
        s_ceps[mem_id][lane] = ceps;
        cg[mem_id * NB_BANDS + lane] = ceps;
        s_feat[lane] = ceps;
    }
    __syncwarp();
    if (lane < NB_DELTA_CEPS) {
        const int c1 = (mem_id < 1) ? CEPS_MEM + mem_id - 1 : mem_id - 1;
        const int c2 = (mem_id < 2) ? CEPS_MEM + mem_id - 2 : mem_id - 2;
        const float a = s_ceps[mem_id][lane], b = s_ceps[c1][lane], c = s_ceps[c2][lane];
        s_feat[lane] = a + b + c;
        s_feat[NB_BANDS + lane] = a - c;
        s_feat[NB_BANDS + NB_DELTA_CEPS + lane] = a - 2.0f * b + c;
        s_feat[NB_BANDS + 2 * NB_DELTA_CEPS + lane] = pcor;
    }
#pragma unroll
    for (int h2 = 0; h2 < 2; h2++) {
        const int pr = lane + 32 * h2, i = pr >> 3, j = pr & 7;
        float dist = 0.0f;
#pragma unroll
        for (int k = 0; k < NB_BANDS; k++) {
            const float t = s_ceps[i][k] - s_ceps[j][k];
            dist += t * t;
        }
        s_dist[i][j] = dist;
    }
    __syncwarp();
    float md = 1e15f;
    if (lane < CEPS_MEM) {
#pragma unroll
        for (int j = 0; j < CEPS_MEM; j++)
            if (j != lane) md = fminf(md, s_dist[lane][j]);
    }
    float sv = 0.0f;
#pragma unroll
    for (int i = 0; i < CEPS_MEM; i++) sv += __shfl_sync(0xffffffffu, md, i);
    if (lane == 0) {
        s_feat[NB_BANDS + 3 * NB_DELTA_CEPS] = 0.01f * ((float)pitch - 300.0f);
        s_feat[NB_BANDS + 3 * NB_DELTA_CEPS + 1] = sv / (float)CEPS_MEM - 2.1f;
        bb.ceps_id[s] = (mem_id + 1 == CEPS_MEM) ? 0 : mem_id + 1;
        bb.silence[s] = 0;
    }
    __syncwarp();
    featg[lane] = s_feat[lane];
    if (lane + 32 < NB_FEATURES) featg[lane + 32] = s_feat[lane + 32];
}

cudaError_t launch_analysis(const BatchBuffers& b, const DeviceTables* tab, int slot, cudaStream_t st) {
    analysis_kernel<<<b.n_streams, ST, 0, st>>>(b, tab, hist_base(slot));
    return cudaGetLastError();
}

__device__ __forceinline__ short to_pcm16(float v) { return (short)roundf(fminf(fmaxf(v, -32768.0f), 32767.0f)); }

template <typename TOut>
__global__ void __launch_bounds__(ST) synthesis_kernel(BatchBuffers bb, const DeviceTables* __restrict__ tab,
                                                       TOut* __restrict__ out, long stream_stride, long sample_stride,
                                                       float* __restrict__ vad_out) {
    __shared__ __align__(16) float2 xs[FREQ_SIZE + 1];
    __shared__ __align__(16) float2 fa_[480];
    __shared__ __align__(16) float2 fb_[480];
    __shared__ float part[BT_LANES];
    __shared__ float s_g[NB_BANDS], s_r[NB_BANDS], s_ne[NB_BANDS], s_ex[NB_BANDS];

    const int s = blockIdx.x, tid = threadIdx.x;
    const float2* Xg = bb.X + (size_t)s * FREQ_SIZE;
    const float2* Pg = bb.P + (size_t)s * NB_BINS_BANDED;
    float2 xv[4], pv[4];
    int bidx[4];
    float bfr[4];
#pragma unroll
    for (int it = 0; it < 4; it++) {
        const int k = tid + it * ST;
        xv[it] = k <= 480 ? __ldg(Xg + k) : make_float2(0.f, 0.f);
        pv[it] = k < NB_BINS_BANDED ? __ldg(Pg + k) : make_float2(0.f, 0.f);
        bidx[it] = k < NB_BINS_BANDED ? __ldg(&tab->band_of[k]) : 0;
        bfr[it] = k < NB_BINS_BANDED ? __ldg(&tab->band_frac[k]) : 0.0f;
    }
    float b_e = 0.f, b_g = 0.f, b_ex = 0.f, b_ep = 0.f, b_lg = 0.f;
    if (tid < NB_BANDS) {
        b_e = bb.exp[(size_t)s * NB_BANDS + tid];
        b_g = bb.gains[(size_t)s * NB_BANDS + tid];
        b_ex = bb.ex[(size_t)s * NB_BANDS + tid];
        b_ep = bb.ep[(size_t)s * NB_BANDS + tid];
        b_lg = bb.lastg[(size_t)s * NB_BANDS + tid];
    }
    const float vad_in = bb.vad[s];
    const int silent = bb.silence[s];
#pragma unroll
    for (int it = 0; it < 4; it++) {
        const int k = tid + it * ST;
        if (k <= 480) xs[k] = xv[it];
    }

    if (!silent) {
        if (tid < NB_BANDS) {
            const float e = b_e, g = b_g, ex = b_ex, ep = b_ep;
            float r;
            if (e > g) {
                r = 1.0f;
            } else {
                float e2 = e * e, g2 = g * g;
                r = e2 * (1.0f - g2) / (0.001f + g2 * (1.0f - e2));
            }
            r = (r < 0.0f) ? 0.0f : r;
            r = (r > 1.0f) ? 1.0f : r;
            r = sqrtf(r);
            r *= sqrtf(ex / (1e-8f + ep));
            s_r[tid] = r;
            s_ex[tid] = ex;
            float gg = fmaxf(g, 0.6f * b_lg);
            s_g[tid] = gg;
            bb.lastg[(size_t)s * NB_BANDS + tid] = gg;
        }
        __syncthreads();
#pragma unroll
        for (int it = 0; it < 4; it++) {
            const int k = tid + it * ST;
            if (k < NB_BINS_BANDED) {
                const float rf = (1.0f - bfr[it]) * s_r[bidx[it]] + bfr[it] * s_r[bidx[it] + 1];
                float2 x = xs[k];
                x.x += pv[it].x * rf;
                if (k > 0) x.y += pv[it].y * rf;
                xs[k] = x;
            }
        }
        __syncthreads();
        band_sums<1>(xs, xs, tab, part, s_ne, s_ne, s_ne);
        if (tid < NB_BANDS) s_r[tid] = sqrtf(s_ex[tid] / (1e-8f + s_ne[tid]));
        __syncthreads();
#pragma unroll
        for (int it = 0; it < 4; it++) {
            const int k = tid + it * ST;
            if (k <= 480) {
                float2 x = xs[k];
                if (k < NB_BINS_BANDED) {
                    const float m1 = (1.0f - bfr[it]) * s_r[bidx[it]] + bfr[it] * s_r[bidx[it] + 1];
                    const float m2 = (1.0f - bfr[it]) * s_g[bidx[it]] + bfr[it] * s_g[bidx[it] + 1];
                    x.x = (x.x * m1) * m2;
                    x.y = (x.y * m1) * m2;
                } else {
                    x = make_float2(0.f, 0.f);
                }
                xs[k] = x;
            }
        }
    }
    __syncthreads();

#pragma unroll
    for (int it = 0; it < 2; it++) {
        const int k = tid + it * ST;
        if (k <= 240) {
            const float2 xk = xs[k], xc = xs[480 - k];
            const float xi = (k == 0) ? 0.0f : xk.y, yi = (k == 0) ? 0.0f : xc.y;
            const float sr = xk.x + xc.x, si = xi - yi;
            const float dr = xk.x - xc.x, di = xi + yi;
            const float2 w = __ldg(&tab->tw960[k]);
            const float tx = dr * w.x + di * w.y, ty = di * w.x - dr * w.y;
            fa_[k] = make_float2(sr - ty, -(si + tx));
            if (k != 0 && k != 240) {
                const float ux = dr * w.x + di * w.y, uy = dr * w.y - di * w.x;
                fa_[480 - k] = make_float2(sr - uy, -(-si + ux));
            }
        }
    }
    __syncthreads();
    fft480(fa_, fb_, tab->tw480);
    float* sm = bb.synth_mem + (size_t)s * FRAME_SIZE;
    TOut* o = out + (long)s * stream_stride;
    const bool o_vec = sample_stride == 1 && ((reinterpret_cast<uintptr_t>(o) & (4 * sizeof(TOut) - 1)) == 0);
    const long ss = sample_stride;
#pragma unroll
    for (int it = 0; it < 2; it++) {
        const int q = tid + it * ST;
        if (q < WINDOW_SIZE / 4) {
            const float4 z = reinterpret_cast<const float4*>(fa_)[q];
            const float4 w = __ldg(reinterpret_cast<const float4*>(tab->window) + q);
            const float4 v = make_float4((z.x * 0.5f) * w.x, (-z.y * 0.5f) * w.y, (z.z * 0.5f) * w.z, (-z.w * 0.5f) * w.w);
            if (q < FRAME_SIZE / 4) {
                const float4 m = reinterpret_cast<const float4*>(sm)[q];
                const float4 r = make_float4(v.x + m.x, v.y + m.y, v.z + m.z, v.w + m.w);
                if (sizeof(TOut) == 4) {
                    float* of = reinterpret_cast<float*>(o);
                    if (o_vec) {
                        reinterpret_cast<float4*>(of)[q] = r;
                    } else {
                        of[(4 * q) * ss] = r.x; of[(4 * q + 1) * ss] = r.y; of[(4 * q + 2) * ss] = r.z; of[(4 * q + 3) * ss] = r.w;
                    }
                } else {
                    short* os = reinterpret_cast<short*>(o);
                    const short p0 = to_pcm16(r.x), p1 = to_pcm16(r.y), p2 = to_pcm16(r.z), p3 = to_pcm16(r.w);
                    if (o_vec) {
                        reinterpret_cast<uint2*>(os)[q] = make_uint2((unsigned)(unsigned short)p0 | ((unsigned)(unsigned short)p1 << 16),
                                                                     (unsigned)(unsigned short)p2 | ((unsigned)(unsigned short)p3 << 16));
                    } else {
                        os[(4 * q) * ss] = p0; os[(4 * q + 1) * ss] = p1; os[(4 * q + 2) * ss] = p2; os[(4 * q + 3) * ss] = p3;
                    }
                }
            } else {
                reinterpret_cast<float4*>(fb_)[q - FRAME_SIZE / 4] = v;
            }
        }
    }
    __syncthreads();
    for (int q = tid; q < FRAME_SIZE / 4; q += ST) reinterpret_cast<float4*>(sm)[q] = reinterpret_cast<const float4*>(fb_)[q];
    if (tid == 0 && vad_out) vad_out[s] = silent ? 0.0f : vad_in;
}

cudaError_t launch_synthesis(const BatchBuffers& b, const DeviceTables* tab, void* out, bool pcm16, long stream_stride, long sample_stride,
                             float* vad_out, cudaStream_t st) {
    if (pcm16) synthesis_kernel<short><<<b.n_streams, ST, 0, st>>>(b, tab, static_cast<short*>(out), stream_stride, sample_stride, vad_out);
    else synthesis_kernel<float><<<b.n_streams, ST, 0, st>>>(b, tab, static_cast<float*>(out), stream_stride, sample_stride, vad_out);
    return cudaGetLastError();
}

}
```

### nnnoiseless_b200/csrc/spectral_warp.cu

```cuda
#include "common.cuh"
#include "fft480.cuh"

namespace nnb {

namespace {

constexpr int WPB = 4;
constexpr int RS = 33;
constexpr int ZP_OFF = 495;
constexpr int WBUF = 30 * RS;
constexpr int SC_SR = 0, SC_SG = 32, SC_SN = 64, SC_BAND = 96;
constexpr int WSC = SC_BAND + 21 * 6 + 2;
static_assert(ZP_OFF + FREQ_SIZE <= WBUF, "two 481-bin spectra must fit the warp buffer");

constexpr int PF_WAVE_A = 132 * 4 * WPB;
__device__ __forceinline__ void prefetch_l2(const void* p) { asm volatile("prefetch.global.L2 [%0];" ::"l"(p)); }

template <bool TWO>
__device__ __forceinline__ void fft480_warp(float2 (&vx)[15], float2 (&vp)[15], float2* __restrict__ buf,
                                            const DeviceTables* __restrict__ tab, int lane) {
    dft15(vx);
    if (TWO) dft15(vp);
#pragma unroll
    for (int k1 = 1; k1 < 15; k1++) {
        const float2 tw = __ldg(&tab->twl[k1][lane]);
        vx[k1] = c_mul(vx[k1], tw);
        if (TWO) vp[k1] = c_mul(vp[k1], tw);
    }
#pragma unroll
    for (int k1 = 0; k1 < 15; k1++) {
        buf[k1 * RS + lane] = vx[k1];
        if (TWO) buf[(15 + k1) * RS + lane] = vp[k1];
    }
    __syncwarp();
    float2 r[32];
    const bool on = lane < (TWO ? 30 : 15);
    if (on) {
#pragma unroll
        for (int b = 0; b < 32; b++) r[b] = buf[lane * RS + b];
        fft32_dif(r);
    }
    __syncwarp();
    if (on) {
        const int base = lane < 15 ? lane : ZP_OFF + lane - 15;
#pragma unroll
        for (int k2 = 0; k2 < 32; k2++) buf[base + 15 * k2] = r[bitrev5(k2)];
    }
    __syncwarp();
}

template <int NQ>
__device__ __forceinline__ void band_sums_warp(const float2* __restrict__ buf, const DeviceTables* __restrict__ tab, float* __restrict__ sc,
                                               int lane, float (&o)[NQ]) {
    const int sg = tab->bp_seg[lane], b0 = tab->bp_b0[lane], n = tab->bp_n[lane], rot = tab->bp_rot[lane], off0 = tab->bp_off[lane];
    const float inv = tab->bp_inv[lane];
    float a[NQ], b[NQ];
#pragma unroll
    for (int q = 0; q < NQ; q++) a[q] = b[q] = 0.0f;
#pragma unroll
    for (int t = 0; t < BP_MAXBINS; t++) {
        if (t < n) {
            int i = t + rot;
            if (i >= n) i -= n;
            const int k = b0 + i;
            const float f = (float)(off0 + i) * inv, g = 1.0f - f;
            const float2 x = buf[k];
            float e[NQ];
            e[0] = x.x * x.x + x.y * x.y;
            if (NQ == 3) {
                const float2 p = buf[ZP_OFF + k];
                e[1] = p.x * p.x + p.y * p.y;
                e[2] = x.x * p.x + x.y * p.y;
            }
#pragma unroll
            for (int q = 0; q < NQ; q++) {
                a[q] = fmaf(g, e[q], a[q]);
                b[q] = fmaf(f, e[q], b[q]);
            }
        }
    }
    {
        float a0[NQ], b0v[NQ];
#pragma unroll
        for (int q = 0; q < NQ; q++) {
            a0[q] = a[q];
            b0v[q] = b[q];
        }
#pragma unroll
        for (int off = 1; off < 4; off++) {
            const int osg = __shfl_down_sync(0xffffffffu, sg, off);
            const bool take = lane + off < 32 && osg == sg;
#pragma unroll
            for (int q = 0; q < NQ; q++) {
                const float va = __shfl_down_sync(0xffffffffu, a0[q], off), vb = __shfl_down_sync(0xffffffffu, b0v[q], off);
                if (take) {
                    a[q] += va;
                    b[q] += vb;
                }
            }
        }
    }
    const int psg = __shfl_up_sync(0xffffffffu, sg, 1);
    if (lane == 0 || psg != sg) {
#pragma unroll
        for (int q = 0; q < NQ; q++) {
            sc[SC_BAND + sg * 6 + q] = a[q];
            sc[SC_BAND + sg * 6 + 3 + q] = b[q];
        }
    }
    __syncwarp();
#pragma unroll
    for (int q = 0; q < NQ; q++) {
        float v = 0.0f;
        if (lane < NB_BANDS) {
            if (lane < NB_BANDS - 1) v = sc[SC_BAND + lane * 6 + q];
            if (lane > 0) v += sc[SC_BAND + (lane - 1) * 6 + 3 + q];
            if (lane == 0 || lane == NB_BANDS - 1) v *= 2.0f;
        }
        o[q] = v;
    }
    __syncwarp();
}

__global__ void __launch_bounds__(WPB * 32, 4) analysis_warp_kernel(BatchBuffers bb, const DeviceTables* __restrict__ tab, int hbase) {
    __shared__ __align__(16) float2 sbuf[WPB][WBUF];
    __shared__ float ssc[WPB][WSC];
    const int lane = threadIdx.x & 31, warp = threadIdx.x >> 5;
    const int s = blockIdx.x * WPB + warp;
    if (s >= bb.n_streams) return;
    float2* buf = sbuf[warp];
    float* sc = ssc[warp];
    const float* h = bb.hist + (size_t)s * HIST_CAP;
    const int pitch = bb.pitch[s];

    float2 vx[15], vp[15];
    {
        int sx = hbase + (PITCH_BUF_SIZE - WINDOW_SIZE);
        if (sx >= HIST_CAP) sx -= HIST_CAP;
        int sp = hbase + (PITCH_BUF_SIZE - WINDOW_SIZE) - pitch;
        if (sp >= HIST_CAP) sp -= HIST_CAP;
        const bool even = (pitch & 1) == 0;
        float2 hx[15], hp[15], wv[15];
#pragma unroll
        for (int a = 0; a < 15; a++) {
            const int n2 = 64 * a + 2 * lane;
            int px = sx + n2;
            if (px >= HIST_CAP) px -= HIST_CAP;
            hx[a] = __ldg(reinterpret_cast<const float2*>(h + px));
            wv[a] = __ldg(reinterpret_cast<const float2*>(tab->window + n2));
            int p0 = sp + n2;
            if (p0 >= HIST_CAP) p0 -= HIST_CAP;
            if (even) {
                hp[a] = __ldg(reinterpret_cast<const float2*>(h + p0));
            } else {
                int p1 = p0 + 1;
                if (p1 >= HIST_CAP) p1 -= HIST_CAP;
                hp[a] = make_float2(__ldg(h + p0), __ldg(h + p1));
            }
        }
        {
            const int sn = s + PF_WAVE_A;
            if (sn < bb.n_streams) {
                const char* hn = reinterpret_cast<const char*>(bb.hist + (size_t)sn * HIST_CAP);
                const char* cn = reinterpret_cast<const char*>(bb.ceps_mem + (size_t)sn * CEPS_MEM * NB_BANDS);
                int o0 = hbase * 4 + 128 * lane;
                if (o0 >= HIST_CAP * 4) o0 -= HIST_CAP * 4;
                prefetch_l2(hn + o0);
                const int l2 = lane + 32;
                if (l2 < 55) {
                    int o1 = hbase * 4 + 128 * l2;
                    if (o1 >= HIST_CAP * 4) o1 -= HIST_CAP * 4;
                    prefetch_l2(hn + o1);
                } else if (l2 < 61) {
                    prefetch_l2(cn + 128 * (l2 - 55));
                } else if (l2 == 61) {
                    prefetch_l2(bb.pitch + sn);
                }
            }
        }
#pragma unroll
        for (int a = 0; a < 15; a++) {
            vx[a] = make_float2(hx[a].x * wv[a].x, hx[a].y * wv[a].y);
            vp[a] = make_float2(hp[a].x * wv[a].x, hp[a].y * wv[a].y);
        }
    }
    fft480_warp<true>(vx, vp, buf, tab, lane);

    {
        const float wn = tab->wnorm;
        float2* Xg = bb.X + (size_t)s * FREQ_SIZE;
        float2* Pg = bb.P + (size_t)s * NB_BINS_BANDED;
#pragma unroll
        for (int j = 0; j < 8; j++) {
            const int k = lane + 32 * j;
            if (k <= 240) {
                const int kc = k == 0 ? 0 : 480 - k;
                const float2 tw = __ldg(&tab->tw960[k]);
                float2 x0, x1, p0, p1;
                rfft_split_pair(buf[k], buf[kc], tw, wn, k == 0, x0, x1);
                rfft_split_pair(buf[ZP_OFF + k], buf[ZP_OFF + kc], tw, wn, k == 0, p0, p1);
                buf[k] = x0;
                buf[ZP_OFF + k] = p0;
                Xg[k] = x0;
                Pg[k] = p0;
                if (k != 240) {
                    buf[480 - k] = x1;
                    buf[ZP_OFF + 480 - k] = p1;
                    Xg[480 - k] = x1;
                    if (480 - k < NB_BINS_BANDED) Pg[480 - k] = p1;
                }
            }
        }
    }
    __syncwarp();

    float bs[3];
    band_sums_warp<3>(buf, tab, sc, lane, bs);

    const bool bl = lane < NB_BANDS;
    const float ex = bs[0], ep = bs[1];
    const float xpn = bl ? bs[2] / sqrtf(0.001f + ex * ep) : 0.0f;
    if (bl) {
        bb.ex[(size_t)s * NB_BANDS + lane] = ex;
        bb.ep[(size_t)s * NB_BANDS + lane] = ep;
        bb.exp[(size_t)s * NB_BANDS + lane] = xpn;
    }
    float* fsc = reinterpret_cast<float*>(buf);
    float* s_ceps = fsc;
    float* s_dist = fsc + CEPS_MEM * NB_BANDS;
    float* s_feat = s_dist + CEPS_MEM * CEPS_MEM;
    float* cg = bb.ceps_mem + (size_t)s * CEPS_MEM * NB_BANDS;
    const int mem_id = bb.ceps_id[s];
    float cr[6];
#pragma unroll
    for (int k = 0; k < 6; k++) cr[k] = (lane + 32 * k < CEPS_MEM * NB_BANDS) ? cg[lane + 32 * k] : 0.0f;
    const float lg = bl ? log10f(1e-2f + ex) : 0.0f;
    float ly = 0.0f, log_max = -2.0f, follow = -2.0f, e = 0.0f;
#pragma unroll
    for (int k = 0; k < NB_BANDS; k++) {
        const float v = fmaxf(fmaxf(__shfl_sync(0xffffffffu, lg, k), log_max - 7.0f), follow - 1.5f);
        if (lane == k) ly = v;
        log_max = fmaxf(log_max, v);
        follow = fmaxf(follow - 1.5f, v);
        e += __shfl_sync(0xffffffffu, ex, k);
    }
    float* featg = bb.features + (size_t)s * NB_FEATURES;
    if (e < 0.04f) {
        featg[lane] = 0.0f;
        if (lane + 32 < NB_FEATURES) featg[lane + 32] = 0.0f;
        if (lane == 0) bb.silence[s] = 1;
        return;
    }
    const double dct_scale = 0.30151134457776362265;
    float sum_ly = 0.0f, sum_xp = 0.0f;
#pragma unroll
    for (int j = 0; j < NB_BANDS; j++) {
        const float d = bl ? __ldg(&tab->dct[j * NB_BANDS + lane]) : 0.0f;
        sum_ly += __shfl_sync(0xffffffffu, ly, j) * d;
        sum_xp += __shfl_sync(0xffffffffu, xpn, j) * d;
    }
    float ceps = (float)((double)sum_ly * dct_scale);
    float pcor = (float)((double)sum_xp * dct_scale);
    if (lane == 0) {
        ceps -= 12.0f;
        pcor -= 1.3f;
    }
    if (lane == 1) {
        ceps -= 4.0f;
        pcor -= 0.9f;
    }
#pragma unroll
    for (int k = 0; k < 6; k++)
        if (lane + 32 * k < CEPS_MEM * NB_BANDS) s_ceps[lane + 32 * k] = cr[k];
    __syncwarp();
    if (bl) {
        s_ceps[mem_id * NB_BANDS + lane] = ceps;
        cg[mem_id * NB_BANDS + lane] = ceps;
        s_feat[lane] = ceps;
    }
    __syncwarp();
    if (lane < NB_DELTA_CEPS) {
        const int c1 = (mem_id < 1) ? CEPS_MEM + mem_id - 1 : mem_id - 1;
        const int c2 = (mem_id < 2) ? CEPS_MEM + mem_id - 2 : mem_id - 2;
        const float a = s_ceps[mem_id * NB_BANDS + lane], b = s_ceps[c1 * NB_BANDS + lane], c = s_ceps[c2 * NB_BANDS + lane];
        s_feat[lane] = a + b + c;
        s_feat[NB_BANDS + lane] = a - c;
        s_feat[NB_BANDS + NB_DELTA_CEPS + lane] = a - 2.0f * b + c;
        s_feat[NB_BANDS + 2 * NB_DELTA_CEPS + lane] = pcor;
    }
#pragma unroll
    for (int h2 = 0; h2 < 2; h2++) {
        const int pr = lane + 32 * h2, i = pr >> 3, j = pr & 7;
        float dist = 0.0f;
#pragma unroll
        for (int k = 0; k < NB_BANDS; k++) {
            const float t = s_ceps[i * NB_BANDS + k] - s_ceps[j * NB_BANDS + k];
            dist += t * t;
        }
        s_dist[i * CEPS_MEM + j] = dist;
    }
    __syncwarp();
    float md = 1e15f;
    if (lane < CEPS_MEM) {
#pragma unroll
        for (int j = 0; j < CEPS_MEM; j++)
            if (j != lane) md = fminf(md, s_dist[lane * CEPS_MEM + j]);
    }
    float sv = 0.0f;
#pragma unroll
    for (int i = 0; i < CEPS_MEM; i++) sv += __shfl_sync(0xffffffffu, md, i);
    if (lane == 0) {
        s_feat[NB_BANDS + 3 * NB_DELTA_CEPS] = 0.01f * ((float)pitch - 300.0f);
        s_feat[NB_BANDS + 3 * NB_DELTA_CEPS + 1] = sv / (float)CEPS_MEM - 2.1f;
        bb.ceps_id[s] = (mem_id + 1 == CEPS_MEM) ? 0 : mem_id + 1;
        bb.silence[s] = 0;
    }
    __syncwarp();
    featg[lane] = s_feat[lane];
    if (lane + 32 < NB_FEATURES) featg[lane + 32] = s_feat[lane + 32];
}

__device__ __forceinline__ short to_pcm16w(float v) { return (short)roundf(fminf(fmaxf(v, -32768.0f), 32767.0f)); }

template <typename TOut>
__global__ void __launch_bounds__(WPB * 32, 4) synthesis_warp_kernel(BatchBuffers bb, const DeviceTables* __restrict__ tab,
                                                                  TOut* __restrict__ out, long stream_stride, long sample_stride,
                                                                  float* __restrict__ vad_out) {
    __shared__ __align__(16) float2 sbuf[WPB][WBUF];
    __shared__ float ssc[WPB][WSC];
    const int lane = threadIdx.x & 31, warp = threadIdx.x >> 5;
    const int s = blockIdx.x * WPB + warp;
    if (s >= bb.n_streams) return;
    float2* buf = sbuf[warp];
    float* sc = ssc[warp];

    const float2* Xg = bb.X + (size_t)s * FREQ_SIZE;
    const float2* Pg = bb.P + (size_t)s * NB_BINS_BANDED;
    float2 xv[16];
#pragma unroll
    for (int j = 0; j < 16; j++) {
        const int k = lane + 32 * j;
        xv[j] = k <= 480 ? __ldg(Xg + k) : make_float2(0.f, 0.f);
    }
    const float vad_in = bb.vad[s];
    const int silent = bb.silence[s];
    float* smem_ola = bb.synth_mem + (size_t)s * FRAME_SIZE;
    float4 ola[4];
#pragma unroll
    for (int j = 0; j < 4; j++) {
        const int q = lane + 32 * j;
        ola[j] = q < FRAME_SIZE / 4 ? __ldg(reinterpret_cast<const float4*>(smem_ola) + q) : make_float4(0.f, 0.f, 0.f, 0.f);
    }
    if (!silent) {
        float2 pv[13];
#pragma unroll
        for (int j = 0; j < 13; j++) {
            const int k = lane + 32 * j;
            pv[j] = k < NB_BINS_BANDED ? __ldg(Pg + k) : make_float2(0.f, 0.f);
        }
        float b_ex = 0.0f;
        if (lane < NB_BANDS) {
            const float e = bb.exp[(size_t)s * NB_BANDS + lane], g = bb.gains[(size_t)s * NB_BANDS + lane];
            const float ex = bb.ex[(size_t)s * NB_BANDS + lane], ep = bb.ep[(size_t)s * NB_BANDS + lane];
            const float lastg = bb.lastg[(size_t)s * NB_BANDS + lane];
            b_ex = ex;
            float r;
            if (e > g) {
                r = 1.0f;
            } else {
                const float e2 = e * e, g2 = g * g;
                r = e2 * (1.0f - g2) / (0.001f + g2 * (1.0f - e2));
            }
            r = (r < 0.0f) ? 0.0f : r;
            r = (r > 1.0f) ? 1.0f : r;
            r = sqrtf(r);
            r *= sqrtf(ex / (1e-8f + ep));
            sc[SC_SR + lane] = r;
            const float gg = fmaxf(g, 0.6f * lastg);
            sc[SC_SG + lane] = gg;
            bb.lastg[(size_t)s * NB_BANDS + lane] = gg;
        }
        __syncwarp();
#pragma unroll
        for (int j = 0; j < 16; j++) {
            const int k = lane + 32 * j;
            if (j < 13 && k < NB_BINS_BANDED) {
                const int bi = __ldg(&tab->band_of[k]);
                const float fr = __ldg(&tab->band_frac[k]);
                const float rf = (1.0f - fr) * sc[SC_SR + bi] + fr * sc[SC_SR + bi + 1];
                xv[j].x += pv[j].x * rf;
                if (k > 0) xv[j].y += pv[j].y * rf;
            }
            if (k <= 480) buf[k] = xv[j];
        }
        __syncwarp();
        float ne[1];
        band_sums_warp<1>(buf, tab, sc, lane, ne);
        if (lane < NB_BANDS) sc[SC_SN + lane] = sqrtf(b_ex / (1e-8f + ne[0]));
        __syncwarp();
#pragma unroll
        for (int j = 0; j < 16; j++) {
            const int k = lane + 32 * j;
            if (k <= 480) {
                float2 x = xv[j];
                if (k < NB_BINS_BANDED) {
                    const int bi = __ldg(&tab->band_of[k]);
                    const float fr = __ldg(&tab->band_frac[k]);
                    const float m1 = (1.0f - fr) * sc[SC_SN + bi] + fr * sc[SC_SN + bi + 1];
                    const float m2 = (1.0f - fr) * sc[SC_SG + bi] + fr * sc[SC_SG + bi + 1];
                    x.x = (x.x * m1) * m2;
                    x.y = (x.y * m1) * m2;
                } else {
                    x = make_float2(0.f, 0.f);
                }
                buf[k] = x;
            }
        }
    } else {
#pragma unroll
        for (int j = 0; j < 16; j++) {
            const int k = lane + 32 * j;
            if (k <= 480) buf[k] = xv[j];
        }
    }
    __syncwarp();

#pragma unroll
    for (int j = 0; j < 8; j++) {
        const int k = lane + 32 * j;
        if (k <= 240) {
            float2 z0, z1;
            irfft_pretwist_pair(buf[k], buf[480 - k], __ldg(&tab->tw960[k]), k == 0, z0, z1);
            buf[k] = z0;
            if (k != 0 && k != 240) buf[480 - k] = z1;
        }
    }
    __syncwarp();
    float2 v[15], dummy[15];
#pragma unroll
    for (int a = 0; a < 15; a++) v[a] = buf[32 * a + lane];
    __syncwarp();
    fft480_warp<false>(v, dummy, buf, tab, lane);

    TOut* o = out + (long)s * stream_stride;
    const bool o_vec = sample_stride == 1 && ((reinterpret_cast<uintptr_t>(o) & (4 * sizeof(TOut) - 1)) == 0);
    const long ss = sample_stride;
#pragma unroll
    for (int j = 0; j < 8; j++) {
        const int q = lane + 32 * j;
        if (q < WINDOW_SIZE / 4) {
            const float4 z = reinterpret_cast<const float4*>(buf)[q];
            const float4 w = __ldg(reinterpret_cast<const float4*>(tab->window) + q);
            const float4 t = make_float4((z.x * 0.5f) * w.x, (-z.y * 0.5f) * w.y, (z.z * 0.5f) * w.z, (-z.w * 0.5f) * w.w);
            if (q < FRAME_SIZE / 4) {
                const float4 m = ola[j < 4 ? j : 0];
                const float4 r = make_float4(t.x + m.x, t.y + m.y, t.z + m.z, t.w + m.w);
                if (sizeof(TOut) == 4) {
                    float* of = reinterpret_cast<float*>(o);
                    if (o_vec) {
                        reinterpret_cast<float4*>(of)[q] = r;
                    } else {
                        of[(4 * q) * ss] = r.x; of[(4 * q + 1) * ss] = r.y; of[(4 * q + 2) * ss] = r.z; of[(4 * q + 3) * ss] = r.w;
                    }
                } else {
                    short* os = reinterpret_cast<short*>(o);
                    const short p0 = to_pcm16w(r.x), p1 = to_pcm16w(r.y), p2 = to_pcm16w(r.z), p3 = to_pcm16w(r.w);
                    if (o_vec) {
                        reinterpret_cast<uint2*>(os)[q] = make_uint2((unsigned)(unsigned short)p0 | ((unsigned)(unsigned short)p1 << 16),
                                                                     (unsigned)(unsigned short)p2 | ((unsigned)(unsigned short)p3 << 16));
                    } else {
                        os[(4 * q) * ss] = p0; os[(4 * q + 1) * ss] = p1; os[(4 * q + 2) * ss] = p2; os[(4 * q + 3) * ss] = p3;
                    }
                }
            } else {
                reinterpret_cast<float4*>(smem_ola)[q - FRAME_SIZE / 4] = t;
            }
        }
    }
    if (lane == 0 && vad_out) vad_out[s] = silent ? 0.0f : vad_in;
}

}

cudaError_t launch_analysis_warp(const BatchBuffers& b, const DeviceTables* tab, int slot, cudaStream_t st) {
    const int grid = (b.n_streams + WPB - 1) / WPB;
    analysis_warp_kernel<<<grid, WPB * 32, 0, st>>>(b, tab, hist_base(slot));
    return cudaGetLastError();
}

cudaError_t launch_synthesis_warp(const BatchBuffers& b, const DeviceTables* tab, void* out, bool pcm16, long stream_stride,
                                  long sample_stride, float* vad_out, cudaStream_t st) {
    const int grid = (b.n_streams + WPB - 1) / WPB;
    if (pcm16) synthesis_warp_kernel<short><<<grid, WPB * 32, 0, st>>>(b, tab, static_cast<short*>(out), stream_stride, sample_stride, vad_out);
    else synthesis_warp_kernel<float><<<grid, WPB * 32, 0, st>>>(b, tab, static_cast<float*>(out), stream_stride, sample_stride, vad_out);
    return cudaGetLastError();
}

}
```

Before: 29.72 million.

## Recompute frame spectra in synthesis instead of storing X/P to global memory

Analysis no longer writes the X and P spectra to global buffers. Synthesis re-derives them from the history ring buffer by running the same windowed FFT and pitch-spectrum routine, with L2 prefetch of the next stream's history and overlap-add memory. This trades extra FFT compute in synthesis for less global write and read traffic. A static_assert checks that the history ring is deep enough that synthesis still sees valid samples while later frames are in flight. The legacy block-wide spectral path and its tables are also removed.

```diff
diff --git a/nnnoiseless_b200/build.py b/nnnoiseless_b200/build.py
--- a/nnnoiseless_b200/build.py
+++ b/nnnoiseless_b200/build.py
@@ -22,7 +22,6 @@
     ("exact.cu", ["-fmad=false"]),
     ("pitch.cu", ["-fmad=false"]),
     ("train.cu", ["-fmad=false"]),
-    ("spectral.cu", []),
     ("spectral_warp.cu", []),
     ("rnn.cu", ["-DRNN_RT=256", "-DRNN_UNROLL=8"]),
     ("rnn_mma.cu", []),
diff --git a/nnnoiseless_b200/csrc/common.cuh b/nnnoiseless_b200/csrc/common.cuh
--- a/nnnoiseless_b200/csrc/common.cuh
+++ b/nnnoiseless_b200/csrc/common.cuh
@@ -17,11 +17,12 @@
 constexpr int NB_FEATURES = 42;
 constexpr int MAX_NEURONS = 128;
 constexpr int NB_BINS_BANDED = 400;
-constexpr int BT_LANES = 96;
 
 constexpr int HIST_SLOTS = 8;
 constexpr int HIST_CAP = HIST_SLOTS * FRAME_SIZE;
 constexpr int PIPE_DEPTH = 4;
+constexpr int HIST_LIVE_SLOTS = (PITCH_BUF_SIZE + FRAME_SIZE - 1) / FRAME_SIZE;
+static_assert(HIST_LIVE_SLOTS + PIPE_DEPTH - 1 <= HIST_SLOTS, "a high-pass kernel in flight would overwrite history that synthesis still reads");
 
 __host__ __device__ inline int hist_base(int slot) { return (slot * FRAME_SIZE + (HIST_CAP - (PITCH_BUF_SIZE - FRAME_SIZE))) % HIST_CAP; }
 
@@ -30,16 +31,10 @@
     float dct[NB_BANDS * NB_BANDS];
     float wnorm;
     float tansig[201 + 3];
-    float2 tw480[480];
     float2 tw960[FREQ_SIZE + 3];
     float band_frac[NB_BINS_BANDED];
     int32_t band_of[NB_BINS_BANDED];
     int32_t band_start[NB_BANDS];
-    int16_t bt_bin[800];
-    float bt_w[800];
-    int16_t bt_lane_start[BT_LANES + 1];
-    int16_t bt_band_lane[NB_BANDS + 1];
-    int16_t bt_lane_band[BT_LANES];
     float2 twl[15][32];
     int16_t bp_seg[32];
     int16_t bp_b0[32];
@@ -91,8 +86,6 @@
     float* last_gain;
     float* gru_state;
     float* lastg;
-    float2* X;
-    float2* P;
     float* ex;
     float* ep;
     float* exp;
@@ -136,11 +129,8 @@
 cudaError_t launch_hp_filter(const BatchBuffers& b, const void* in, bool pcm16, long stream_stride, long sample_stride, int slot,
                              cudaStream_t st);
 cudaError_t launch_pitch(const BatchBuffers& b, int slot, int force_exact, cudaStream_t st);
-cudaError_t launch_analysis(const BatchBuffers& b, const DeviceTables* tab, int slot, cudaStream_t st);
-cudaError_t launch_synthesis(const BatchBuffers& b, const DeviceTables* tab, void* out, bool pcm16, long stream_stride, long sample_stride,
-                             float* vad_out, cudaStream_t st);
 cudaError_t launch_analysis_warp(const BatchBuffers& b, const DeviceTables* tab, int slot, cudaStream_t st);
-cudaError_t launch_synthesis_warp(const BatchBuffers& b, const DeviceTables* tab, void* out, bool pcm16, long stream_stride,
+cudaError_t launch_synthesis_warp(const BatchBuffers& b, const DeviceTables* tab, int slot, void* out, bool pcm16, long stream_stride,
                                   long sample_stride, float* vad_out, cudaStream_t st);
 cudaError_t launch_rnn(const BatchBuffers& b, const DeviceModel& m, const DeviceTables* tab, cudaStream_t st);
 cudaError_t launch_rnn_mma(const BatchBuffers& b, const DeviceModelMma& m, const DeviceTables* tab, cudaStream_t st);
diff --git a/nnnoiseless_b200/csrc/host.cu b/nnnoiseless_b200/csrc/host.cu
--- a/nnnoiseless_b200/csrc/host.cu
+++ b/nnnoiseless_b200/csrc/host.cu
@@ -101,8 +101,6 @@
             t->dct[i * NB_BANDS + j] = v;
         }
     for (int i = 0; i < 201; i++) t->tansig[i] = kTansigTable[i];
-    for (int k = 0; k < 480; k++)
-        t->tw480[k] = make_float2((float)std::cos(-2.0 * pi * (double)k / 480.0), (float)std::sin(-2.0 * pi * (double)k / 480.0));
     for (int k = 0; k <= 480; k++)
         t->tw960[k] = make_float2((float)std::cos(-2.0 * pi * (double)k / 960.0), (float)std::sin(-2.0 * pi * (double)k / 960.0));
     for (int i = 0; i < NB_BANDS; i++) t->band_start[i] = kEband5ms[i] << 2;
@@ -112,26 +110,6 @@
             int idx = (kEband5ms[i] << 2) + j;
             t->band_frac[idx] = (float)j / (float)band_size;
             t->band_of[idx] = i;
-        }
-    }
-    int nterm = 0, lane = 0;
-    for (int b = 0; b < NB_BANDS; b++) {
-        const int first = nterm;
-        if (b > 0)
-            for (int i = t->band_start[b - 1]; i < t->band_start[b]; i++) {
-                t->bt_bin[nterm] = (int16_t)i;
-                t->bt_w[nterm++] = t->band_frac[i];
-            }
-        if (b < NB_BANDS - 1)
-            for (int i = t->band_start[b]; i < t->band_start[b + 1]; i++) {
-                t->bt_bin[nterm] = (int16_t)i;
-                t->bt_w[nterm++] = 1.0f - t->band_frac[i];
-            }
-        const int n = nterm - first, lanes = (n + 8) / 9;
-        t->bt_band_lane[b] = (int16_t)lane;
-        for (int l = 0; l < lanes; l++) {
-            t->bt_lane_band[lane] = (int16_t)b;
-            t->bt_lane_start[lane++] = (int16_t)(first + (int)((long)n * l / lanes));
         }
     }
     for (int k1 = 0; k1 < 15; k1++)
@@ -164,12 +142,6 @@
             fprintf(stderr, "nnnoiseless_b200: band partition uses %d lanes\n", l);
             abort();
         }
-    }
-    t->bt_band_lane[NB_BANDS] = (int16_t)lane;
-    t->bt_lane_start[lane] = (int16_t)nterm;
-    if (lane != BT_LANES || nterm != 800) {
-        fprintf(stderr, "nnnoiseless_b200: band table construction broken (%d lanes, %d terms)\n", lane, nterm);
-        abort();
     }
 }
 
@@ -386,7 +358,6 @@
     UploadedTc utc;
     bool rnn_mma = false;
     bool rnn_fp32 = false;
-    bool spectral_v1 = false;
     bool serial = false;
     int pitch_exact = 0;
     unsigned long long frame = 0;
@@ -413,8 +384,6 @@
 BatchBuffers view(const RNNoiseBatch* b, unsigned long long f) {
     BatchBuffers v = b->buf;
     const size_t k = (size_t)(f % PIPE_DEPTH), B = (size_t)b->n_streams;
-    v.X += k * B * FREQ_SIZE;
-    v.P += k * B * NB_BINS_BANDED;
     v.ex += k * B * NB_BANDS;
     v.ep += k * B * NB_BANDS;
     v.exp += k * B * NB_BANDS;
@@ -493,8 +462,6 @@
         b->serial = e2 && e2[0] == '1';
         const char* e5 = getenv("NNB_RNN_MMA");
         b->rnn_mma = e5 && e5[0] == '1';
-        const char* e4 = getenv("NNB_SPECTRAL_V1");
-        b->spectral_v1 = e4 && e4[0] == '1';
         const char* e3 = getenv("NNB_PITCH_EXACT");
         b->pitch_exact = !e3 ? 0 : (e3[0] == '1' ? 3 : (e3[0] == '2' ? 1 : (e3[0] == '3' ? 2 : 0)));
     }
@@ -502,7 +469,7 @@
     if (dalloc(b, &u.hist, B * HIST_CAP) || dalloc(b, &u.hp_mem, B * 2) || dalloc(b, &u.synth_mem, B * FRAME_SIZE) ||
         dalloc(b, &u.ceps_mem, B * CEPS_MEM * NB_BANDS) || dalloc(b, &u.ceps_id, B) || dalloc(b, &u.last_period, B) ||
         dalloc(b, &u.last_gain, B) || dalloc(b, &u.gru_state, B * SS) || dalloc(b, &u.lastg, B * NB_BANDS) ||
-        dalloc(b, &u.X, D * B * FREQ_SIZE) || dalloc(b, &u.P, D * B * NB_BINS_BANDED) || dalloc(b, &u.ex, D * B * NB_BANDS) ||
+        dalloc(b, &u.ex, D * B * NB_BANDS) ||
         dalloc(b, &u.ep, D * B * NB_BANDS) || dalloc(b, &u.exp, D * B * NB_BANDS) || dalloc(b, &u.features, D * B * NB_FEATURES) ||
         dalloc(b, &u.silence, D * B) || dalloc(b, &u.pitch, D * B) || dalloc(b, &u.gains, D * B * NB_BANDS) ||
         dalloc(b, &u.vad, D * B) || dalloc(b, &b->d_tab, 1) || dalloc(b, &u.pitch_stats, 3))
@@ -573,19 +540,13 @@
     switch (i) {
         case 0: CK(launch_hp_filter(v, in, (fmt & kFmtPcmIn) != 0, stream_stride, sample_stride, slot, s)); break;
         case 1: CK(launch_pitch(v, slot, b->pitch_exact, s)); break;
-        case 2:
-            if (b->spectral_v1) CK(launch_analysis(v, b->d_tab, slot, s));
-            else CK(launch_analysis_warp(v, b->d_tab, slot, s));
-            break;
+        case 2: CK(launch_analysis_warp(v, b->d_tab, slot, s)); break;
         case 3:
             if (b->rnn_fp32) CK(launch_rnn(v, b->um.dm, b->d_tab, s));
             else if (b->utc.ok && !b->rnn_mma) CK(launch_rnn_tc(v, b->utc, s));
             else CK(launch_rnn_mma(v, b->umm.dm, b->d_tab, s));
             break;
-        default:
-            if (b->spectral_v1) CK(launch_synthesis(v, b->d_tab, out, (fmt & kFmtPcmOut) != 0, stream_stride, sample_stride, vad, s));
-            else CK(launch_synthesis_warp(v, b->d_tab, out, (fmt & kFmtPcmOut) != 0, stream_stride, sample_stride, vad, s));
-            break;
+        default: CK(launch_synthesis_warp(v, b->d_tab, slot, out, (fmt & kFmtPcmOut) != 0, stream_stride, sample_stride, vad, s)); break;
     }
     return 0;
 }
@@ -940,10 +901,7 @@
         switch (i) {
             case 0: CK(launch_train_front(v, t->tb, set, sig, noise, stream_stride, slot, S(i))); break;
             case 1: CK(launch_pitch(v, slot, b->pitch_exact, S(i))); break;
-            case 2:
-                if (b->spectral_v1) CK(launch_analysis(v, b->d_tab, slot, S(i)));
-                else CK(launch_analysis_warp(v, b->d_tab, slot, S(i)));
-                break;
+            case 2: CK(launch_analysis_warp(v, b->d_tab, slot, S(i))); break;
             default: CK(launch_train_rows(v, t->tb, set, rows, row_lane_stride, S(i))); break;
         }
         CK(cudaEventRecord(b->ev[i][e], S(i)));
diff --git a/nnnoiseless_b200/csrc/spectral.cu b/nnnoiseless_b200/csrc/spectral.cu
--- a/nnnoiseless_b200/csrc/spectral.cu
+++ /dev/null
@@ -1,577 +0,0 @@
-#include "common.cuh"
-
-namespace nnb {
-
-constexpr int ST = 128;
-
-__device__ __forceinline__ float2 cmul(float2 a, float2 b) { return make_float2(a.x * b.x - a.y * b.y, a.x * b.y + a.y * b.x); }
-__device__ __forceinline__ float2 cadd(float2 a, float2 b) { return make_float2(a.x + b.x, a.y + b.y); }
-__device__ __forceinline__ float2 csub(float2 a, float2 b) { return make_float2(a.x - b.x, a.y - b.y); }
-
-template <int R>
-__device__ __forceinline__ void butterfly(float2* a) {
-    if (R == 2) {
-        float2 t = a[0];
-        a[0] = cadd(t, a[1]);
-        a[1] = csub(t, a[1]);
-    } else if (R == 4) {
-        float2 t0 = cadd(a[0], a[2]), t1 = csub(a[0], a[2]);
-        float2 t2 = cadd(a[1], a[3]), t3 = csub(a[1], a[3]);
-        a[0] = cadd(t0, t2);
-        a[1] = make_float2(t1.x + t3.y, t1.y - t3.x);
-        a[2] = csub(t0, t2);
-        a[3] = make_float2(t1.x - t3.y, t1.y + t3.x);
-    } else if (R == 3) {
-        const float s = 0.86602540378443864676f;
-        float2 t1 = cadd(a[1], a[2]), d = csub(a[1], a[2]);
-        float2 m1 = make_float2(a[0].x - 0.5f * t1.x, a[0].y - 0.5f * t1.y);
-        a[0] = cadd(a[0], t1);
-        a[1] = make_float2(m1.x + s * d.y, m1.y - s * d.x);
-        a[2] = make_float2(m1.x - s * d.y, m1.y + s * d.x);
-    } else if (R == 6) {
-        const float h = 0.5f, s = 0.86602540378443864676f;
-        float2 e[3] = {a[0], a[2], a[4]}, o[3] = {a[1], a[3], a[5]};
-        butterfly<3>(e);
-        butterfly<3>(o);
-        const float2 t1 = make_float2(h * o[1].x + s * o[1].y, h * o[1].y - s * o[1].x);
-        const float2 t2 = make_float2(s * o[2].y - h * o[2].x, -h * o[2].y - s * o[2].x);
-        a[0] = cadd(e[0], o[0]);
-        a[3] = csub(e[0], o[0]);
-        a[1] = cadd(e[1], t1);
-        a[4] = csub(e[1], t1);
-        a[2] = cadd(e[2], t2);
-        a[5] = csub(e[2], t2);
-    } else if (R == 5) {
-        const float c1 = 0.30901699437494742410f, c2 = -0.80901699437494742410f;
-        const float s1 = 0.95105651629515357212f, s2 = 0.58778525229247312917f;
-        float2 t1 = cadd(a[1], a[4]), t2 = cadd(a[2], a[3]);
-        float2 d1 = csub(a[1], a[4]), d2 = csub(a[2], a[3]);
-        float2 u1 = make_float2(a[0].x + c1 * t1.x + c2 * t2.x, a[0].y + c1 * t1.y + c2 * t2.y);
-        float2 u2 = make_float2(a[0].x + c2 * t1.x + c1 * t2.x, a[0].y + c2 * t1.y + c1 * t2.y);
-        float2 v1 = make_float2(s1 * d1.x + s2 * d2.x, s1 * d1.y + s2 * d2.y);
-        float2 v2 = make_float2(s2 * d1.x - s1 * d2.x, s2 * d1.y - s1 * d2.y);
-        a[0] = cadd(a[0], cadd(t1, t2));
-        a[1] = make_float2(u1.x + v1.y, u1.y - v1.x);
-        a[4] = make_float2(u1.x - v1.y, u1.y + v1.x);
-        a[2] = make_float2(u2.x + v2.y, u2.y - v2.x);
-        a[3] = make_float2(u2.x - v2.y, u2.y + v2.x);
-    }
-}
-
-template <int R, int N, int S>
-__device__ __forceinline__ void stockham_pass(const float2* __restrict__ x, float2* __restrict__ y,
-                                              const float2* __restrict__ tw) {
-    constexpr int M = N / R;
-    for (int b = threadIdx.x; b < 480 / R; b += ST) {
-        const int p = b / S, q = b - p * S;
-        float2 a[R];
-#pragma unroll
-        for (int k = 0; k < R; k++) a[k] = x[q + S * (p + k * M)];
-        butterfly<R>(a);
-        y[q + S * (R * p)] = a[0];
-#pragma unroll
-        for (int j = 1; j < R; j++) {
-            y[q + S * (R * p + j)] = (N == R) ? a[j] : cmul(a[j], __ldg(&tw[j * p * S]));
-        }
-    }
-    __syncthreads();
-}
-
-__device__ void fft480(float2* a, float2* b, const float2* tw) {
-    stockham_pass<4, 480, 1>(a, b, tw);
-    stockham_pass<4, 120, 4>(b, a, tw);
-    stockham_pass<5, 30, 16>(a, b, tw);
-    stockham_pass<6, 6, 80>(b, a, tw);
-}
-
-template <int R, int N, int S>
-__device__ __forceinline__ void stockham_pass2(const float2* __restrict__ x0, float2* __restrict__ y0, const float2* __restrict__ x1,
-                                               float2* __restrict__ y1, const float2* __restrict__ tw) {
-    constexpr int M = N / R;
-    for (int b = threadIdx.x; b < 480 / R; b += ST) {
-        const int p = b / S, q = b - p * S;
-        float2 a[R], c[R];
-#pragma unroll
-        for (int k = 0; k < R; k++) {
-            a[k] = x0[q + S * (p + k * M)];
-            c[k] = x1[q + S * (p + k * M)];
-        }
-        butterfly<R>(a);
-        butterfly<R>(c);
-        y0[q + S * (R * p)] = a[0];
-        y1[q + S * (R * p)] = c[0];
-#pragma unroll
-        for (int j = 1; j < R; j++) {
-            if (N == R) {
-                y0[q + S * (R * p + j)] = a[j];
-                y1[q + S * (R * p + j)] = c[j];
-            } else {
-                const float2 w = __ldg(&tw[j * p * S]);
-                y0[q + S * (R * p + j)] = cmul(a[j], w);
-                y1[q + S * (R * p + j)] = cmul(c[j], w);
-            }
-        }
-    }
-    __syncthreads();
-}
-__device__ void fft480x2(float2* a0, float2* b0, float2* a1, float2* b1, const float2* tw) {
-    stockham_pass2<4, 480, 1>(a0, b0, a1, b1, tw);
-    stockham_pass2<4, 120, 4>(b0, a0, b1, a1, tw);
-    stockham_pass2<5, 30, 16>(a0, b0, a1, b1, tw);
-    stockham_pass2<6, 6, 80>(b0, a0, b1, a1, tw);
-}
-
-template <int NS>
-__device__ __forceinline__ void band_sums(const float2* xs, const float2* ps, const DeviceTables* __restrict__ tab, float* part,
-                                          float* o0, float* o1, float* o2) {
-    const int tid = threadIdx.x, lane = tid & 31, warp = tid >> 5;
-    static_assert(BT_LANES == 96, "three warps of band lanes");
-    if (tid < BT_LANES) {
-        const int t0 = tab->bt_lane_start[tid], n = tab->bt_lane_start[tid + 1] - t0;
-        const int bin0 = tab->bt_bin[t0];
-        const int band = tab->bt_lane_band[tid];
-        float a0 = 0.0f, a1 = 0.0f, a2 = 0.0f;
-#pragma unroll
-        for (int i = 0; i < 9; i++) {
-            if (i < n) {
-                const float w = __ldg(&tab->bt_w[t0 + i]);
-                const float2 x = xs[bin0 + i];
-                a0 = fmaf(w, x.x * x.x + x.y * x.y, a0);
-                if (NS == 3) {
-                    const float2 p = ps[bin0 + i];
-                    a1 = fmaf(w, p.x * p.x + p.y * p.y, a1);
-                    a2 = fmaf(w, x.x * p.x + x.y * p.y, a2);
-                }
-            }
-        }
-#pragma unroll
-        for (int off = 1; off < 32; off <<= 1) {
-            const int ob = __shfl_down_sync(0xffffffffu, band, off);
-            const float v0 = __shfl_down_sync(0xffffffffu, a0, off);
-            const float v1 = NS == 3 ? __shfl_down_sync(0xffffffffu, a1, off) : 0.0f;
-            const float v2 = NS == 3 ? __shfl_down_sync(0xffffffffu, a2, off) : 0.0f;
-            if (lane + off < 32 && ob == band) {
-                a0 += v0;
-                if (NS == 3) {
-                    a1 += v1;
-                    a2 += v2;
-                }
-            }
-        }
-        const int prev = __shfl_up_sync(0xffffffffu, band, 1);
-        if (lane == 0 || prev != band) {
-            part[warp * NB_BANDS + band] = a0;
-            if (NS == 3) {
-                part[(3 + warp) * NB_BANDS + band] = a1;
-                part[(6 + warp) * NB_BANDS + band] = a2;
-            }
-        }
-    }
-    __syncthreads();
-    if (tid < NS * 32) {
-        const int which = tid >> 5, b = tid & 31;
-        if (b < NB_BANDS) {
-            const int w0 = tab->bt_band_lane[b] >> 5, w1 = (tab->bt_band_lane[b + 1] - 1) >> 5;
-            float acc = 0.0f;
-            for (int w = w0; w <= w1; w++) acc += part[(which * 3 + w) * NB_BANDS + b];
-            if (b == 0 || b == NB_BANDS - 1) acc *= 2.0f;
-            float* o = which == 0 ? o0 : (which == 1 ? o1 : o2);
-            o[b] = acc;
-        }
-    }
-    __syncthreads();
-}
-
-__device__ __forceinline__ float interp_gain(const float* g, const DeviceTables* __restrict__ tab, int idx) {
-    if (idx >= NB_BINS_BANDED) return 0.0f;
-    int b = tab->band_of[idx];
-    float f = tab->band_frac[idx];
-    return (1.0f - f) * g[b] + f * g[b + 1];
-}
-
-struct WindowLoad {
-    float4 hv[2], wv[2];
-    float2 hs[4], ws[4];
-    bool aligned;
-    __device__ __forceinline__ void issue_loads(const float* __restrict__ h, int start, const DeviceTables* __restrict__ tab) {
-        aligned = (start & 3) == 0;
-        if (aligned) {
-#pragma unroll
-            for (int it = 0; it < 2; it++) {
-                const int q = threadIdx.x + it * ST;
-                hv[it] = make_float4(0.f, 0.f, 0.f, 0.f);
-                wv[it] = hv[it];
-                if (q < WINDOW_SIZE / 4) {
-                    int pos = start + 4 * q;
-                    if (pos >= HIST_CAP) pos -= HIST_CAP;
-                    hv[it] = __ldg(reinterpret_cast<const float4*>(h + pos));
-                    wv[it] = __ldg(reinterpret_cast<const float4*>(tab->window) + q);
-                }
-            }
-        } else {
-#pragma unroll
-            for (int it = 0; it < 4; it++) {
-                const int n = threadIdx.x + it * ST;
-                hs[it] = make_float2(0.f, 0.f);
-                ws[it] = hs[it];
-                if (n < 480) {
-                    int p0 = start + 2 * n;
-                    if (p0 >= HIST_CAP) p0 -= HIST_CAP;
-                    int p1 = p0 + 1;
-                    if (p1 >= HIST_CAP) p1 -= HIST_CAP;
-                    hs[it] = make_float2(__ldg(h + p0), __ldg(h + p1));
-                    ws[it] = __ldg(reinterpret_cast<const float2*>(tab->window) + n);
-                }
-            }
-        }
-    }
-    __device__ __forceinline__ void store(float2* a) const {
-        if (aligned) {
-#pragma unroll
-            for (int it = 0; it < 2; it++) {
-                const int q = threadIdx.x + it * ST;
-                if (q < WINDOW_SIZE / 4)
-                    reinterpret_cast<float4*>(a)[q] = make_float4(hv[it].x * wv[it].x, hv[it].y * wv[it].y, hv[it].z * wv[it].z, hv[it].w * wv[it].w);
-            }
-        } else {
-#pragma unroll
-            for (int it = 0; it < 4; it++) {
-                const int n = threadIdx.x + it * ST;
-                if (n < 480) a[n] = make_float2(hs[it].x * ws[it].x, hs[it].y * ws[it].y);
-            }
-        }
-    }
-};
-
-__device__ __forceinline__ void rfft_post(const float2* b, float2* xs, const DeviceTables* __restrict__ tab) {
-    const float wn = tab->wnorm;
-#pragma unroll
-    for (int it = 0; it < 2; it++) {
-        const int k = threadIdx.x + it * ST;
-        if (k <= 240) {
-            const float2 zk = b[k], zc = b[k == 0 ? 0 : 480 - k];
-            const float er = 0.5f * (zk.x + zc.x), ei = 0.5f * (zk.y - zc.y);
-            const float dr = 0.5f * (zk.x - zc.x), di = 0.5f * (zk.y + zc.y);
-            const float2 tw = __ldg(&tab->tw960[k]);
-            const float tx = di * tw.x + dr * tw.y, ty = di * tw.y - dr * tw.x;
-            float2 r0 = make_float2((er + tx) * wn, (ei + ty) * wn);
-            float2 r1 = make_float2((er - tx) * wn, (ty - ei) * wn);
-            if (k == 0) {
-                r0.y = 0.0f;
-                r1.y = 0.0f;
-            }
-            xs[k] = r0;
-            if (k != 240) xs[480 - k] = r1;
-        }
-    }
-}
-
-__global__ void __launch_bounds__(ST, 10) analysis_kernel(BatchBuffers bb, const DeviceTables* __restrict__ tab, int hbase) {
-    __shared__ __align__(16) float2 xa[FREQ_SIZE + 1];
-    __shared__ __align__(16) float2 xb[480];
-    __shared__ __align__(16) float2 pa[FREQ_SIZE + 1];
-    __shared__ __align__(16) float2 pb[480];
-    __shared__ float part[3 * BT_LANES];
-    __shared__ float s_ex[NB_BANDS], s_ep[NB_BANDS], s_exp[NB_BANDS];
-    __shared__ float s_feat[NB_FEATURES];
-    __shared__ float s_ceps[CEPS_MEM][NB_BANDS];
-    __shared__ float s_dist[CEPS_MEM][CEPS_MEM];
-
-    const int s = blockIdx.x, tid = threadIdx.x;
-    const float* h = bb.hist + (size_t)s * HIST_CAP;
-    const int pitch = bb.pitch[s];
-
-    int start = hbase + (PITCH_BUF_SIZE - WINDOW_SIZE);
-    if (start >= HIST_CAP) start -= HIST_CAP;
-    WindowLoad wx, wp;
-    wx.issue_loads(h, start, tab);
-    start = hbase + (PITCH_BUF_SIZE - WINDOW_SIZE) - pitch;
-    if (start >= HIST_CAP) start -= HIST_CAP;
-    wp.issue_loads(h, start, tab);
-    wx.store(xa);
-    wp.store(pa);
-    __syncthreads();
-    fft480x2(xa, xb, pa, pb, tab->tw480);
-    float2* xs = xa;
-    float2* ps = pa;
-    rfft_post(xa, xs, tab);
-    rfft_post(pa, ps, tab);
-    __syncthreads();
-
-    float2* Xg = bb.X + (size_t)s * FREQ_SIZE;
-    float2* Pg = bb.P + (size_t)s * NB_BINS_BANDED;
-    for (int k = tid; k <= 480; k += ST) Xg[k] = xs[k];
-    for (int k = tid; k < NB_BINS_BANDED; k += ST) Pg[k] = ps[k];
-    band_sums<3>(xs, ps, tab, part, s_ex, s_ep, s_exp);
-
-    if (tid >= 32) return;
-    const int lane = tid;
-    const bool bl = lane < NB_BANDS;
-    const float ex = bl ? s_ex[lane] : 0.0f, ep = bl ? s_ep[lane] : 0.0f;
-    const float xpn = bl ? s_exp[lane] / sqrtf(0.001f + ex * ep) : 0.0f;
-    if (bl) {
-        bb.ex[(size_t)s * NB_BANDS + lane] = ex;
-        bb.ep[(size_t)s * NB_BANDS + lane] = ep;
-        bb.exp[(size_t)s * NB_BANDS + lane] = xpn;
-    }
-    float* cg = bb.ceps_mem + (size_t)s * CEPS_MEM * NB_BANDS;
-    const int mem_id = bb.ceps_id[s];
-    float cr[6];
-#pragma unroll
-    for (int k = 0; k < 6; k++) cr[k] = (lane + 32 * k < CEPS_MEM * NB_BANDS) ? cg[lane + 32 * k] : 0.0f;
-    const float lg = bl ? log10f(1e-2f + ex) : 0.0f;
-    float ly = 0.0f, log_max = -2.0f, follow = -2.0f, e = 0.0f;
-#pragma unroll
-    for (int k = 0; k < NB_BANDS; k++) {
-        const float v = fmaxf(fmaxf(__shfl_sync(0xffffffffu, lg, k), log_max - 7.0f), follow - 1.5f);
-        if (lane == k) ly = v;
-        log_max = fmaxf(log_max, v);
-        follow = fmaxf(follow - 1.5f, v);
-        e += __shfl_sync(0xffffffffu, ex, k);
-    }
-    float* featg = bb.features + (size_t)s * NB_FEATURES;
-    if (e < 0.04f) {
-        featg[lane] = 0.0f;
-        if (lane + 32 < NB_FEATURES) featg[lane + 32] = 0.0f;
-        if (lane == 0) bb.silence[s] = 1;
-        return;
-    }
-    const double dct_scale = 0.30151134457776362265;
-    float sum_ly = 0.0f, sum_xp = 0.0f;
-#pragma unroll
-    for (int j = 0; j < NB_BANDS; j++) {
-        const float d = bl ? __ldg(&tab->dct[j * NB_BANDS + lane]) : 0.0f;
-        sum_ly += __shfl_sync(0xffffffffu, ly, j) * d;
-        sum_xp += __shfl_sync(0xffffffffu, xpn, j) * d;
-    }
-    float ceps = (float)((double)sum_ly * dct_scale);
-    float pcor = (float)((double)sum_xp * dct_scale);
-    if (lane == 0) {
-        ceps -= 12.0f;
-        pcor -= 1.3f;
-    }
-    if (lane == 1) {
-        ceps -= 4.0f;
-        pcor -= 0.9f;
-    }
-#pragma unroll
-    for (int k = 0; k < 6; k++)
-        if (lane + 32 * k < CEPS_MEM * NB_BANDS) (&s_ceps[0][0])[lane + 32 * k] = cr[k];
-    __syncwarp();
-    if (bl) {
-        s_ceps[mem_id][lane] = ceps;
-        cg[mem_id * NB_BANDS + lane] = ceps;
-        s_feat[lane] = ceps;
-    }
-    __syncwarp();
-    if (lane < NB_DELTA_CEPS) {
-        const int c1 = (mem_id < 1) ? CEPS_MEM + mem_id - 1 : mem_id - 1;
-        const int c2 = (mem_id < 2) ? CEPS_MEM + mem_id - 2 : mem_id - 2;
-        const float a = s_ceps[mem_id][lane], b = s_ceps[c1][lane], c = s_ceps[c2][lane];
-        s_feat[lane] = a + b + c;
-        s_feat[NB_BANDS + lane] = a - c;
-        s_feat[NB_BANDS + NB_DELTA_CEPS + lane] = a - 2.0f * b + c;
-        s_feat[NB_BANDS + 2 * NB_DELTA_CEPS + lane] = pcor;
-    }
-#pragma unroll
-    for (int h2 = 0; h2 < 2; h2++) {
-        const int pr = lane + 32 * h2, i = pr >> 3, j = pr & 7;
-        float dist = 0.0f;
-#pragma unroll
-        for (int k = 0; k < NB_BANDS; k++) {
-            const float t = s_ceps[i][k] - s_ceps[j][k];
-            dist += t * t;
-        }
-        s_dist[i][j] = dist;
-    }
-    __syncwarp();
-    float md = 1e15f;
-    if (lane < CEPS_MEM) {
-#pragma unroll
-        for (int j = 0; j < CEPS_MEM; j++)
-            if (j != lane) md = fminf(md, s_dist[lane][j]);
-    }
-    float sv = 0.0f;
-#pragma unroll
-    for (int i = 0; i < CEPS_MEM; i++) sv += __shfl_sync(0xffffffffu, md, i);
-    if (lane == 0) {
-        s_feat[NB_BANDS + 3 * NB_DELTA_CEPS] = 0.01f * ((float)pitch - 300.0f);
-        s_feat[NB_BANDS + 3 * NB_DELTA_CEPS + 1] = sv / (float)CEPS_MEM - 2.1f;
-        bb.ceps_id[s] = (mem_id + 1 == CEPS_MEM) ? 0 : mem_id + 1;
-        bb.silence[s] = 0;
-    }
-    __syncwarp();
-    featg[lane] = s_feat[lane];
-    if (lane + 32 < NB_FEATURES) featg[lane + 32] = s_feat[lane + 32];
-}
-
-cudaError_t launch_analysis(const BatchBuffers& b, const DeviceTables* tab, int slot, cudaStream_t st) {
-    analysis_kernel<<<b.n_streams, ST, 0, st>>>(b, tab, hist_base(slot));
-    return cudaGetLastError();
-}
-
-__device__ __forceinline__ short to_pcm16(float v) { return (short)roundf(fminf(fmaxf(v, -32768.0f), 32767.0f)); }
-
-template <typename TOut>
-__global__ void __launch_bounds__(ST) synthesis_kernel(BatchBuffers bb, const DeviceTables* __restrict__ tab,
-                                                       TOut* __restrict__ out, long stream_stride, long sample_stride,
-                                                       float* __restrict__ vad_out) {
-    __shared__ __align__(16) float2 xs[FREQ_SIZE + 1];
-    __shared__ __align__(16) float2 fa_[480];
-    __shared__ __align__(16) float2 fb_[480];
-    __shared__ float part[BT_LANES];
-    __shared__ float s_g[NB_BANDS], s_r[NB_BANDS], s_ne[NB_BANDS], s_ex[NB_BANDS];
-
-    const int s = blockIdx.x, tid = threadIdx.x;
-    const float2* Xg = bb.X + (size_t)s * FREQ_SIZE;
-    const float2* Pg = bb.P + (size_t)s * NB_BINS_BANDED;
-    float2 xv[4], pv[4];
-    int bidx[4];
-    float bfr[4];
-#pragma unroll
-    for (int it = 0; it < 4; it++) {
-        const int k = tid + it * ST;
-        xv[it] = k <= 480 ? __ldg(Xg + k) : make_float2(0.f, 0.f);
-        pv[it] = k < NB_BINS_BANDED ? __ldg(Pg + k) : make_float2(0.f, 0.f);
-        bidx[it] = k < NB_BINS_BANDED ? __ldg(&tab->band_of[k]) : 0;
-        bfr[it] = k < NB_BINS_BANDED ? __ldg(&tab->band_frac[k]) : 0.0f;
-    }
-    float b_e = 0.f, b_g = 0.f, b_ex = 0.f, b_ep = 0.f, b_lg = 0.f;
-    if (tid < NB_BANDS) {
-        b_e = bb.exp[(size_t)s * NB_BANDS + tid];
-        b_g = bb.gains[(size_t)s * NB_BANDS + tid];
-        b_ex = bb.ex[(size_t)s * NB_BANDS + tid];
-        b_ep = bb.ep[(size_t)s * NB_BANDS + tid];
-        b_lg = bb.lastg[(size_t)s * NB_BANDS + tid];
-    }
-    const float vad_in = bb.vad[s];
-    const int silent = bb.silence[s];
-#pragma unroll
-    for (int it = 0; it < 4; it++) {
-        const int k = tid + it * ST;
-        if (k <= 480) xs[k] = xv[it];
-    }
-
-    if (!silent) {
-        if (tid < NB_BANDS) {
-            const float e = b_e, g = b_g, ex = b_ex, ep = b_ep;
-            float r;
-            if (e > g) {
-                r = 1.0f;
-            } else {
-                float e2 = e * e, g2 = g * g;
-                r = e2 * (1.0f - g2) / (0.001f + g2 * (1.0f - e2));
-            }
-            r = (r < 0.0f) ? 0.0f : r;
-            r = (r > 1.0f) ? 1.0f : r;
-            r = sqrtf(r);
-            r *= sqrtf(ex / (1e-8f + ep));
-            s_r[tid] = r;
-            s_ex[tid] = ex;
-            float gg = fmaxf(g, 0.6f * b_lg);
-            s_g[tid] = gg;
-            bb.lastg[(size_t)s * NB_BANDS + tid] = gg;
-        }
-        __syncthreads();
-#pragma unroll
-        for (int it = 0; it < 4; it++) {
-            const int k = tid + it * ST;
-            if (k < NB_BINS_BANDED) {
-                const float rf = (1.0f - bfr[it]) * s_r[bidx[it]] + bfr[it] * s_r[bidx[it] + 1];
-                float2 x = xs[k];
-                x.x += pv[it].x * rf;
-                if (k > 0) x.y += pv[it].y * rf;
-                xs[k] = x;
-            }
-        }
-        __syncthreads();
-        band_sums<1>(xs, xs, tab, part, s_ne, s_ne, s_ne);
-        if (tid < NB_BANDS) s_r[tid] = sqrtf(s_ex[tid] / (1e-8f + s_ne[tid]));
-        __syncthreads();
-#pragma unroll
-        for (int it = 0; it < 4; it++) {
-            const int k = tid + it * ST;
-            if (k <= 480) {
-                float2 x = xs[k];
-                if (k < NB_BINS_BANDED) {
-                    const float m1 = (1.0f - bfr[it]) * s_r[bidx[it]] + bfr[it] * s_r[bidx[it] + 1];
-                    const float m2 = (1.0f - bfr[it]) * s_g[bidx[it]] + bfr[it] * s_g[bidx[it] + 1];
-                    x.x = (x.x * m1) * m2;
-                    x.y = (x.y * m1) * m2;
-                } else {
-                    x = make_float2(0.f, 0.f);
-                }
-                xs[k] = x;
-            }
-        }
-    }
-    __syncthreads();
-
-#pragma unroll
-    for (int it = 0; it < 2; it++) {
-        const int k = tid + it * ST;
-        if (k <= 240) {
-            const float2 xk = xs[k], xc = xs[480 - k];
-            const float xi = (k == 0) ? 0.0f : xk.y, yi = (k == 0) ? 0.0f : xc.y;
-            const float sr = xk.x + xc.x, si = xi - yi;
-            const float dr = xk.x - xc.x, di = xi + yi;
-            const float2 w = __ldg(&tab->tw960[k]);
-            const float tx = dr * w.x + di * w.y, ty = di * w.x - dr * w.y;
-            fa_[k] = make_float2(sr - ty, -(si + tx));
-            if (k != 0 && k != 240) {
-                const float ux = dr * w.x + di * w.y, uy = dr * w.y - di * w.x;
-                fa_[480 - k] = make_float2(sr - uy, -(-si + ux));
-            }
-        }
-    }
-    __syncthreads();
-    fft480(fa_, fb_, tab->tw480);
-    float* sm = bb.synth_mem + (size_t)s * FRAME_SIZE;
-    TOut* o = out + (long)s * stream_stride;
-    const bool o_vec = sample_stride == 1 && ((reinterpret_cast<uintptr_t>(o) & (4 * sizeof(TOut) - 1)) == 0);
-    const long ss = sample_stride;
-#pragma unroll
-    for (int it = 0; it < 2; it++) {
-        const int q = tid + it * ST;
-        if (q < WINDOW_SIZE / 4) {
-            const float4 z = reinterpret_cast<const float4*>(fa_)[q];
-            const float4 w = __ldg(reinterpret_cast<const float4*>(tab->window) + q);
-            const float4 v = make_float4((z.x * 0.5f) * w.x, (-z.y * 0.5f) * w.y, (z.z * 0.5f) * w.z, (-z.w * 0.5f) * w.w);
-            if (q < FRAME_SIZE / 4) {
-                const float4 m = reinterpret_cast<const float4*>(sm)[q];
-                const float4 r = make_float4(v.x + m.x, v.y + m.y, v.z + m.z, v.w + m.w);
-                if (sizeof(TOut) == 4) {
-                    float* of = reinterpret_cast<float*>(o);
-                    if (o_vec) {
-                        reinterpret_cast<float4*>(of)[q] = r;
-                    } else {
-                        of[(4 * q) * ss] = r.x; of[(4 * q + 1) * ss] = r.y; of[(4 * q + 2) * ss] = r.z; of[(4 * q + 3) * ss] = r.w;
-                    }
-                } else {
-                    short* os = reinterpret_cast<short*>(o);
-                    const short p0 = to_pcm16(r.x), p1 = to_pcm16(r.y), p2 = to_pcm16(r.z), p3 = to_pcm16(r.w);
-                    if (o_vec) {
-                        reinterpret_cast<uint2*>(os)[q] = make_uint2((unsigned)(unsigned short)p0 | ((unsigned)(unsigned short)p1 << 16),
-                                                                     (unsigned)(unsigned short)p2 | ((unsigned)(unsigned short)p3 << 16));
-                    } else {
-                        os[(4 * q) * ss] = p0; os[(4 * q + 1) * ss] = p1; os[(4 * q + 2) * ss] = p2; os[(4 * q + 3) * ss] = p3;
-                    }
-                }
-            } else {
-                reinterpret_cast<float4*>(fb_)[q - FRAME_SIZE / 4] = v;
-            }
-        }
-    }
-    __syncthreads();
-    for (int q = tid; q < FRAME_SIZE / 4; q += ST) reinterpret_cast<float4*>(sm)[q] = reinterpret_cast<const float4*>(fb_)[q];
-    if (tid == 0 && vad_out) vad_out[s] = silent ? 0.0f : vad_in;
-}
-
-cudaError_t launch_synthesis(const BatchBuffers& b, const DeviceTables* tab, void* out, bool pcm16, long stream_stride, long sample_stride,
-                             float* vad_out, cudaStream_t st) {
-    if (pcm16) synthesis_kernel<short><<<b.n_streams, ST, 0, st>>>(b, tab, static_cast<short*>(out), stream_stride, sample_stride, vad_out);
-    else synthesis_kernel<float><<<b.n_streams, ST, 0, st>>>(b, tab, static_cast<float*>(out), stream_stride, sample_stride, vad_out);
-    return cudaGetLastError();
-}
-
-}
diff --git a/nnnoiseless_b200/csrc/spectral_warp.cu b/nnnoiseless_b200/csrc/spectral_warp.cu
--- a/nnnoiseless_b200/csrc/spectral_warp.cu
+++ b/nnnoiseless_b200/csrc/spectral_warp.cu
@@ -122,17 +122,9 @@
     __syncwarp();
 }
 
-__global__ void __launch_bounds__(WPB * 32, 4) analysis_warp_kernel(BatchBuffers bb, const DeviceTables* __restrict__ tab, int hbase) {
-    __shared__ __align__(16) float2 sbuf[WPB][WBUF];
-    __shared__ float ssc[WPB][WSC];
-    const int lane = threadIdx.x & 31, warp = threadIdx.x >> 5;
-    const int s = blockIdx.x * WPB + warp;
-    if (s >= bb.n_streams) return;
-    float2* buf = sbuf[warp];
-    float* sc = ssc[warp];
-    const float* h = bb.hist + (size_t)s * HIST_CAP;
-    const int pitch = bb.pitch[s];
-
+template <typename Prefetch>
+__device__ __forceinline__ void frame_spectra_warp(const float* __restrict__ h, const DeviceTables* __restrict__ tab, int hbase, int pitch,
+                                                   float2* __restrict__ buf, int lane, Prefetch&& prefetch_next) {
     float2 vx[15], vp[15];
     {
         int sx = hbase + (PITCH_BUF_SIZE - WINDOW_SIZE);
@@ -158,26 +150,7 @@
                 hp[a] = make_float2(__ldg(h + p0), __ldg(h + p1));
             }
         }
-        {
-            const int sn = s + PF_WAVE_A;
-            if (sn < bb.n_streams) {
-                const char* hn = reinterpret_cast<const char*>(bb.hist + (size_t)sn * HIST_CAP);
-                const char* cn = reinterpret_cast<const char*>(bb.ceps_mem + (size_t)sn * CEPS_MEM * NB_BANDS);
-                int o0 = hbase * 4 + 128 * lane;
-                if (o0 >= HIST_CAP * 4) o0 -= HIST_CAP * 4;
-                prefetch_l2(hn + o0);
-                const int l2 = lane + 32;
-                if (l2 < 55) {
-                    int o1 = hbase * 4 + 128 * l2;
-                    if (o1 >= HIST_CAP * 4) o1 -= HIST_CAP * 4;
-                    prefetch_l2(hn + o1);
-                } else if (l2 < 61) {
-                    prefetch_l2(cn + 128 * (l2 - 55));
-                } else if (l2 == 61) {
-                    prefetch_l2(bb.pitch + sn);
-                }
-            }
-        }
+        prefetch_next();
 #pragma unroll
         for (int a = 0; a < 15; a++) {
             vx[a] = make_float2(hx[a].x * wv[a].x, hx[a].y * wv[a].y);
@@ -186,33 +159,57 @@
     }
     fft480_warp<true>(vx, vp, buf, tab, lane);
 
-    {
-        const float wn = tab->wnorm;
-        float2* Xg = bb.X + (size_t)s * FREQ_SIZE;
-        float2* Pg = bb.P + (size_t)s * NB_BINS_BANDED;
-#pragma unroll
-        for (int j = 0; j < 8; j++) {
-            const int k = lane + 32 * j;
-            if (k <= 240) {
-                const int kc = k == 0 ? 0 : 480 - k;
-                const float2 tw = __ldg(&tab->tw960[k]);
-                float2 x0, x1, p0, p1;
-                rfft_split_pair(buf[k], buf[kc], tw, wn, k == 0, x0, x1);
-                rfft_split_pair(buf[ZP_OFF + k], buf[ZP_OFF + kc], tw, wn, k == 0, p0, p1);
-                buf[k] = x0;
-                buf[ZP_OFF + k] = p0;
-                Xg[k] = x0;
-                Pg[k] = p0;
-                if (k != 240) {
-                    buf[480 - k] = x1;
-                    buf[ZP_OFF + 480 - k] = p1;
-                    Xg[480 - k] = x1;
-                    if (480 - k < NB_BINS_BANDED) Pg[480 - k] = p1;
-                }
-            }
-        }
-    }
-    __syncwarp();
+    const float wn = tab->wnorm;
+#pragma unroll
+    for (int j = 0; j < 8; j++) {
+        const int k = lane + 32 * j;
+        if (k <= 240) {
+            const int kc = k == 0 ? 0 : 480 - k;
+            const float2 tw = __ldg(&tab->tw960[k]);
+            float2 x0, x1, p0, p1;
+            rfft_split_pair(buf[k], buf[kc], tw, wn, k == 0, x0, x1);
+            rfft_split_pair(buf[ZP_OFF + k], buf[ZP_OFF + kc], tw, wn, k == 0, p0, p1);
+            buf[k] = x0;
+            buf[ZP_OFF + k] = p0;
+            if (k != 240) {
+                buf[480 - k] = x1;
+                buf[ZP_OFF + 480 - k] = p1;
+            }
+        }
+    }
+    __syncwarp();
+}
+
+__global__ void __launch_bounds__(WPB * 32, 4) analysis_warp_kernel(BatchBuffers bb, const DeviceTables* __restrict__ tab, int hbase) {
+    __shared__ __align__(16) float2 sbuf[WPB][WBUF];
+    __shared__ float ssc[WPB][WSC];
+    const int lane = threadIdx.x & 31, warp = threadIdx.x >> 5;
+    const int s = blockIdx.x * WPB + warp;
+    if (s >= bb.n_streams) return;
+    float2* buf = sbuf[warp];
+    float* sc = ssc[warp];
+    const int pitch = bb.pitch[s];
+
+    frame_spectra_warp(bb.hist + (size_t)s * HIST_CAP, tab, hbase, pitch, buf, lane, [&] {
+        const int sn = s + PF_WAVE_A;
+        if (sn < bb.n_streams) {
+            const char* hn = reinterpret_cast<const char*>(bb.hist + (size_t)sn * HIST_CAP);
+            const char* cn = reinterpret_cast<const char*>(bb.ceps_mem + (size_t)sn * CEPS_MEM * NB_BANDS);
+            int o0 = hbase * 4 + 128 * lane;
+            if (o0 >= HIST_CAP * 4) o0 -= HIST_CAP * 4;
+            prefetch_l2(hn + o0);
+            const int l2 = lane + 32;
+            if (l2 < 55) {
+                int o1 = hbase * 4 + 128 * l2;
+                if (o1 >= HIST_CAP * 4) o1 -= HIST_CAP * 4;
+                prefetch_l2(hn + o1);
+            } else if (l2 < 61) {
+                prefetch_l2(cn + 128 * (l2 - 55));
+            } else if (l2 == 61) {
+                prefetch_l2(bb.pitch + sn);
+            }
+        }
+    });
 
     float bs[3];
     band_sums_warp<3>(buf, tab, sc, lane, bs);
@@ -323,7 +320,7 @@
 __device__ __forceinline__ short to_pcm16w(float v) { return (short)roundf(fminf(fmaxf(v, -32768.0f), 32767.0f)); }
 
 template <typename TOut>
-__global__ void __launch_bounds__(WPB * 32, 4) synthesis_warp_kernel(BatchBuffers bb, const DeviceTables* __restrict__ tab,
+__global__ void __launch_bounds__(WPB * 32, 4) synthesis_warp_kernel(BatchBuffers bb, const DeviceTables* __restrict__ tab, int hbase,
                                                                   TOut* __restrict__ out, long stream_stride, long sample_stride,
                                                                   float* __restrict__ vad_out) {
     __shared__ __align__(16) float2 sbuf[WPB][WBUF];
@@ -334,14 +331,27 @@
     float2* buf = sbuf[warp];
     float* sc = ssc[warp];
 
-    const float2* Xg = bb.X + (size_t)s * FREQ_SIZE;
-    const float2* Pg = bb.P + (size_t)s * NB_BINS_BANDED;
-    float2 xv[16];
-#pragma unroll
-    for (int j = 0; j < 16; j++) {
-        const int k = lane + 32 * j;
-        xv[j] = k <= 480 ? __ldg(Xg + k) : make_float2(0.f, 0.f);
-    }
+    const int pitch = bb.pitch[s];
+    const int sn = s + PF_WAVE_A;
+    const int pitch_n = sn < bb.n_streams ? bb.pitch[sn] : 0;
+    frame_spectra_warp(bb.hist + (size_t)s * HIST_CAP, tab, hbase, pitch, buf, lane, [&] {
+        if (sn < bb.n_streams) {
+            const char* hn = reinterpret_cast<const char*>(bb.hist + (size_t)sn * HIST_CAP);
+            const char* on = reinterpret_cast<const char*>(bb.synth_mem + (size_t)sn * FRAME_SIZE);
+            const int l0 = (PITCH_BUF_SIZE - WINDOW_SIZE - pitch_n) * 4 / 128, nh = PITCH_BUF_SIZE * 4 / 128 - l0;
+#pragma unroll
+            for (int r = 0; r < 3; r++) {
+                const int l = lane + 32 * r;
+                if (l < nh) {
+                    int o = hbase * 4 + 128 * (l0 + l);
+                    if (o >= HIST_CAP * 4) o -= HIST_CAP * 4;
+                    prefetch_l2(hn + o);
+                } else if (l < nh + FRAME_SIZE * 4 / 128) {
+                    prefetch_l2(on + 128 * (l - nh));
+                }
+            }
+        }
+    });
     const float vad_in = bb.vad[s];
     const int silent = bb.silence[s];
     float* smem_ola = bb.synth_mem + (size_t)s * FRAME_SIZE;
@@ -352,12 +362,6 @@
         ola[j] = q < FRAME_SIZE / 4 ? __ldg(reinterpret_cast<const float4*>(smem_ola) + q) : make_float4(0.f, 0.f, 0.f, 0.f);
     }
     if (!silent) {
-        float2 pv[13];
-#pragma unroll
-        for (int j = 0; j < 13; j++) {
-            const int k = lane + 32 * j;
-            pv[j] = k < NB_BINS_BANDED ? __ldg(Pg + k) : make_float2(0.f, 0.f);
-        }
         float b_ex = 0.0f;
         if (lane < NB_BANDS) {
             const float e = bb.exp[(size_t)s * NB_BANDS + lane], g = bb.gains[(size_t)s * NB_BANDS + lane];
@@ -382,16 +386,18 @@
         }
         __syncwarp();
 #pragma unroll
-        for (int j = 0; j < 16; j++) {
+        for (int j = 0; j < 13; j++) {
             const int k = lane + 32 * j;
-            if (j < 13 && k < NB_BINS_BANDED) {
+            if (k < NB_BINS_BANDED) {
                 const int bi = __ldg(&tab->band_of[k]);
                 const float fr = __ldg(&tab->band_frac[k]);
                 const float rf = (1.0f - fr) * sc[SC_SR + bi] + fr * sc[SC_SR + bi + 1];
-                xv[j].x += pv[j].x * rf;
-                if (k > 0) xv[j].y += pv[j].y * rf;
-            }
-            if (k <= 480) buf[k] = xv[j];
+                const float2 p = buf[ZP_OFF + k];
+                float2 x = buf[k];
+                x.x += p.x * rf;
+                if (k > 0) x.y += p.y * rf;
+                buf[k] = x;
+            }
         }
         __syncwarp();
         float ne[1];
@@ -402,25 +408,18 @@
         for (int j = 0; j < 16; j++) {
             const int k = lane + 32 * j;
             if (k <= 480) {
-                float2 x = xv[j];
+                float2 x = make_float2(0.f, 0.f);
                 if (k < NB_BINS_BANDED) {
+                    x = buf[k];
                     const int bi = __ldg(&tab->band_of[k]);
                     const float fr = __ldg(&tab->band_frac[k]);
                     const float m1 = (1.0f - fr) * sc[SC_SN + bi] + fr * sc[SC_SN + bi + 1];
                     const float m2 = (1.0f - fr) * sc[SC_SG + bi] + fr * sc[SC_SG + bi + 1];
                     x.x = (x.x * m1) * m2;
                     x.y = (x.y * m1) * m2;
-                } else {
-                    x = make_float2(0.f, 0.f);
                 }
                 buf[k] = x;
             }
-        }
-    } else {
-#pragma unroll
-        for (int j = 0; j < 16; j++) {
-            const int k = lane + 32 * j;
-            if (k <= 480) buf[k] = xv[j];
         }
     }
     __syncwarp();
@@ -488,11 +487,11 @@
     return cudaGetLastError();
 }
 
-cudaError_t launch_synthesis_warp(const BatchBuffers& b, const DeviceTables* tab, void* out, bool pcm16, long stream_stride,
+cudaError_t launch_synthesis_warp(const BatchBuffers& b, const DeviceTables* tab, int slot, void* out, bool pcm16, long stream_stride,
                                   long sample_stride, float* vad_out, cudaStream_t st) {
-    const int grid = (b.n_streams + WPB - 1) / WPB;
-    if (pcm16) synthesis_warp_kernel<short><<<grid, WPB * 32, 0, st>>>(b, tab, static_cast<short*>(out), stream_stride, sample_stride, vad_out);
-    else synthesis_warp_kernel<float><<<grid, WPB * 32, 0, st>>>(b, tab, static_cast<float*>(out), stream_stride, sample_stride, vad_out);
+    const int grid = (b.n_streams + WPB - 1) / WPB, hbase = hist_base(slot);
+    if (pcm16) synthesis_warp_kernel<short><<<grid, WPB * 32, 0, st>>>(b, tab, hbase, static_cast<short*>(out), stream_stride, sample_stride, vad_out);
+    else synthesis_warp_kernel<float><<<grid, WPB * 32, 0, st>>>(b, tab, hbase, static_cast<float*>(out), stream_stride, sample_stride, vad_out);
     return cudaGetLastError();
 }
 
```

Result: no change. 29.61 million, median of 6 (-0.4%).
